# mp3guy/ElasticFusion

Hardware: AMD Instinct MI355X
Metric: frames/s per GPU, 640x480 3-level ICP+fuse (higher is better)
Workload: dtype f32

## Files before the change

### elasticfusion_amd/api.py

```python
from __future__ import annotations

import ctypes as C
import os
import re

import numpy as np

_HERE = os.path.dirname(os.path.abspath(__file__))
LIB_PATH = os.environ.get("EF_HIP_LIB") or os.path.join(_HERE, "libefusion_hip.so")
_lib = None

c_f, c_i, c_u32, P = C.c_float, C.c_int, C.c_uint32, C.c_void_p


class EFError(RuntimeError):
    pass


class ef_config(C.Structure):
    _fields_ = [("width", c_i), ("height", c_i), ("fx", c_f), ("fy", c_f), ("cx", c_f), ("cy", c_f),
                ("time_delta", c_i), ("confidence", c_f), ("depth_cut", c_f), ("icp_weight", c_f),
                ("fast_odom", c_i), ("so3", c_i), ("frame_to_frame_rgb", c_i), ("pyramid", c_i), ("rgb_only", c_i),
                ("close_loops", c_i), ("max_surfels", c_u32), ("device", c_i), ("stream", P)]

# ... 1521 lines not shown
        return tmp.to_array(np.float32, (h, w, 4)), vm.to_array(np.float32, (3 * h, w)), nm.to_array(np.float32, (3 * h, w))

    @staticmethod
    def resize_map(src, normalize, init=None):
        h3, w = src.shape
        s = DevBuf.from_array(src)
        o = DevBuf.from_array(np.zeros((h3 // 2, w // 2), np.float32) if init is None else init)
        fn = lib().ef_op_resize_nmap if normalize else lib().ef_op_resize_vmap
        _chk(fn(s.p, w, h3 // 3, o.p, None))
        return o.to_array(np.float32, (h3 // 2, w // 2))

    @staticmethod
    def pyr_down_gauss_f(src):
        return ops._image_op("pyr_down_gauss_f", src, np.float32, 2)

    @staticmethod
    def pyr_down_uchar_gauss(src):
        return ops._image_op("pyr_down_uchar_gauss", src, np.uint8, 2)

    @staticmethod
    def vertices_to_depth(vmaps_tmp, cutoff):
        return ops._image_op("vertices_to_depth", ops._f32(vmaps_tmp), np.float32, 1, cutoff)

    @staticmethod
    def bgr_to_intensity(rgba):
        return ops._image_op("image_bgr_to_intensity", rgba, np.uint8, 1)

    @staticmethod
    def derivative_images(img):
        h, w = img.shape
        s, dx, dy = DevBuf.from_array(img), DevBuf(h * w * 2), DevBuf(h * w * 2)
        _chk(lib().ef_op_compute_derivative_images(s.p, w, h, dx.p, dy.p, None))
        return dx.to_array(np.int16, (h, w)), dy.to_array(np.int16, (h, w))

    @staticmethod
    def project_to_point_cloud(depth, fx, fy, cx, cy, level=0):
        h, w = depth.shape
        s, d = DevBuf.from_array(depth), DevBuf(h * w * 12)
        k = ef_intr(fx, fy, cx, cy)
        _chk(lib().ef_op_project_to_point_cloud(s.p, w, h, C.byref(k), level, d.p, None))
        return d.to_array(np.float32, (h, w, 3))

    @staticmethod
    def icp_step(Rcurr, tcurr, vmap_curr, nmap_curr, Rprev_inv, tprev, intr, vmap_g_prev, nmap_g_prev, distThres, angleThres):
        h3, w = vmap_curr.shape
        bufs = [DevBuf.from_array(a) for a in (vmap_curr, nmap_curr, vmap_g_prev, nmap_g_prev)]
        A, b, res = np.zeros((6, 6), np.float32), np.zeros(6, np.float32), np.zeros(2, np.float32)
        k = ef_intr(*intr)
        _chk(lib().ef_op_icp_step(_ptr(ops._f32(Rcurr).reshape(9)), _ptr(ops._f32(tcurr)), bufs[0].p, bufs[1].p,
                                  _ptr(ops._f32(Rprev_inv).reshape(9)), _ptr(ops._f32(tprev)), C.byref(k), bufs[2].p, bufs[3].p,
                                  distThres, angleThres, w, h3 // 3, _ptr(A), _ptr(b), _ptr(res), None))
        return A, b, res

    @staticmethod
    def rgb_residual(minScale, dIdx, dIdy, lastDepth, nextDepth, lastImage, nextImage, maxDepthDelta, kt, krkinv):
        h, w = nextImage.shape
        bufs = [DevBuf.from_array(a) for a in (dIdx, dIdy, lastDepth, nextDepth, lastImage, nextImage)]
        corres = DevBuf(h * w * 16)
        sigma, count = c_i(0), c_i(0)
        _chk(lib().ef_op_compute_rgb_residual(minScale, bufs[0].p, bufs[1].p, bufs[2].p, bufs[3].p, bufs[4].p, bufs[5].p, corres.p,
                                              maxDepthDelta, _ptr(ops._f32(kt)), _ptr(ops._f32(krkinv).reshape(9)), w, h,
                                              C.byref(sigma), C.byref(count), None))
        return corres.to_array(DATATERM, (h, w)), sigma.value, count.value

    @staticmethod
    def rgb_step(corres, sigma, cloud, fx, fy, dIdx, dIdy, sobelScale):
        h, w = corres.shape
        bufs = [DevBuf.from_array(a) for a in (corres, ops._f32(cloud), dIdx, dIdy)]
        A, b = np.zeros((6, 6), np.float32), np.zeros(6, np.float32)
        _chk(lib().ef_op_rgb_step(bufs[0].p, sigma, bufs[1].p, fx, fy, bufs[2].p, bufs[3].p, sobelScale, w, h,
                                  _ptr(A), _ptr(b), None))
        return A, b

    @staticmethod
    def so3_step(lastImage, nextImage, imageBasis, kinv, krlr):
        h, w = nextImage.shape
        li, ni = DevBuf.from_array(lastImage), DevBuf.from_array(nextImage)
        A, b, res = np.zeros((3, 3), np.float32), np.zeros(3, np.float32), np.zeros(2, np.float32)
        _chk(lib().ef_op_so3_step(li.p, ni.p, _ptr(ops._f32(imageBasis).reshape(9)), _ptr(ops._f32(kinv).reshape(9)),
                                  _ptr(ops._f32(krlr).reshape(9)), w, h, _ptr(A), _ptr(b), _ptr(res), None))
        return A, b, res

    @staticmethod
    def model_maps(pred_vertex, pred_normal, fill_vertex, fill_normal, R, t, maxDepthRGB=6.0, pred_image=None, fill_image=None, camera_frame=False,
                   force_fill_image=False, tally=False, dense_count=0, dense_samples=1, joint=False, raw=None, rgb=None, depth_cut=3.0, init=None):
        h, w, _ = pred_vertex.shape
        init = init or {}
        keep = [DevBuf.from_array(ops._f32(a)) for a in (pred_vertex, pred_normal, fill_vertex, fill_normal)]
        a = ef_model_maps_op()
        a.cols, a.rows = w, h
        a.pred_vertex, a.pred_normal, a.fill_vertex, a.fill_normal = (b.p for b in keep)
        if pred_image is not None:
            imgs = [DevBuf.from_array(np.ascontiguousarray(i, np.uint8)) for i in (pred_image, fill_image)]
            keep += imgs
            a.pred_image, a.fill_image = imgs[0].p, imgs[1].p
        a.R[:] = [float(v) for v in ops._f32(R).reshape(9)]
        a.t[:] = [float(v) for v in ops._f32(t).reshape(3)]
        a.max_depth_rgb = float(maxDepthRGB)
        a.camera_frame, a.force_fill_image, a.tally = int(camera_frame), int(force_fill_image), int(tally)
        a.dense_count, a.dense_samples = int(dense_count), int(dense_samples)
        spec = {}
        for l in range(3):
            spec[f"vmap{l}"] = spec[f"nmap{l}"] = (np.float32, (3 * (h >> l), w >> l))
        spec["depth0"], spec["last0"] = (np.float32, (h, w)), (np.uint8, (h, w))
        if joint:
            spec.update(filtered=(np.uint16, (h, w)), metric=(np.float32, (h, w)), metric_filtered=(np.float32, (h, w)), next0=(np.uint8, (h, w)))
        out = {}
        for name, (dt, shp) in spec.items():
            start = np.zeros(shp, dt) if name not in init else np.ascontiguousarray(init[name], dt)
            assert start.shape == shp, (name, start.shape, shp)
            out[name] = DevBuf.from_array(start)
        for l in range(3):
            a.vmap[l], a.nmap[l] = out[f"vmap{l}"].p, out[f"nmap{l}"].p
        a.depth0, a.last0 = out["depth0"].p, out["last0"].p
        if joint:
            fr = [DevBuf.from_array(np.ascontiguousarray(raw, np.uint16)), DevBuf.from_array(np.ascontiguousarray(rgb, np.uint8))]
            assert raw.shape == (h, w) and rgb.shape == (h, w, 3)
            keep += fr
            a.joint, a.raw, a.rgb3, a.depth_cut = 1, fr[0].p, fr[1].p, float(depth_cut)
            a.filtered, a.metric, a.metric_filtered, a.next0 = (out[n].p for n in ("filtered", "metric", "metric_filtered", "next0"))
        left = C.c_uint(0)
        _chk(lib().ef_op_model_maps(C.byref(a), C.byref(left), None))
        res = {name: out[name].to_array(*spec[name]) for name in spec}
        res["dense_count"] = int(left.value)
        return res

    @staticmethod
    def sobel_mask(nextImage, nextDepth):
        h, w = nextImage[0].shape
        img = [DevBuf.from_array(np.ascontiguousarray(a, np.uint8)) for a in nextImage]
        dep = [DevBuf.from_array(ops._f32(a)) for a in nextDepth]
        for l in range(3):
            assert nextImage[l].shape == nextDepth[l].shape == (h >> l, w >> l), (l, nextImage[l].shape, nextDepth[l].shape)
        outs = [[DevBuf((h >> l) * (w >> l) * sz, fill=0xA5) for l in range(3)] for sz in (2, 2, 1, 4)]
        arr = lambda bufs: (P * 3)(*[b.p for b in bufs])
        _chk(lib().ef_op_sobel_mask(arr(img), arr(dep), w, h, arr(outs[0]), arr(outs[1]), arr(outs[2]), arr(outs[3]), None))
        return tuple([b.to_array(dt, (h >> l, w >> l)) for l, b in enumerate(bufs)] for bufs, dt in zip(outs, (np.int16, np.int16, np.uint8, np.uint32)))

    @staticmethod
    def clean_deform(cam, T_wc, time, idx, vc, ct, nr, confThreshold, timeDelta, maxDepth, surfels, newUnstable, graph, depth, isFern=0):
        s = ops._f32(surfels).reshape(-1, 12)
        nu = ops._f32(newUnstable).reshape(-1, 12)
        g = ops._f32(graph).reshape(-1, 16)
        bufs = [DevBuf.from_array(a) for a in (idx, ops._f32(vc), ops._f32(ct), ops._f32(nr), g, ops._f32(depth))]
        sb, nb = DevBuf.from_array(s), DevBuf.from_array(nu if len(nu) else np.zeros((1, 12), np.float32))
        out = DevBuf((len(s) + len(nu) + 1) * 48)
        n = c_u32(0)
        _chk(lib().ef_op_clean_deform(C.byref(cam), _ptr(ops._T(T_wc)), time, bufs[0].p, bufs[1].p, bufs[2].p, bufs[3].p,
                                      confThreshold, timeDelta, maxDepth, sb.p, len(s), nb.p, len(nu),
                                      bufs[4].p, len(g), bufs[5].p, int(isFern), out.p, C.byref(n), None))
        return out.to_array(np.float32, (n.value, 12))

    LINALG = dict(ldlt6=0, ldlt3f=1, polar3=2, rodrigues=3, se3_inverse=4, se3_log_norm=5, scalar=6, ldlt6_wave=7, ldlt6_every_lane=8,
                  mat_to_quat=9, se3_mul=10, se3_castf=11, se3_inverse_f=12, m4_affine_inverse=13, ldlt_pivots=14, lu_inverse6=15)

    @staticmethod
    def linalg(which, vec, n_out):
        v = np.ascontiguousarray(np.asarray(vec, np.float64).reshape(-1))
        out = np.zeros(n_out, np.float64)
        _chk(lib().ef_op_linalg(ops.LINALG[which], _ptr(v), v.size, _ptr(out), n_out))
        return out

    GN_STATE = ("Rcurr", "tcurr", "resultRt", "krkinv", "kt", "lastRGBErrorLevel", "rgb_broken")

    @staticmethod
    def gn_update(sums, prev, Rprev, tprev, count, sigma, icp, rgb, rgbOnly, icpWeight, knext, level_changes, split_tail, lastA, lastb, stats):
        a = ef_gn_update_args()
        a.sums[:] = [float(v) for v in ops._f32(sums).reshape(58)]
        for name in ("Rcurr", "tcurr", "krkinv", "kt"):
            getattr(a.prev, name)[:] = [float(v) for v in ops._f32(prev[name]).reshape(-1)]
        a.prev.resultRt[:] = [float(v) for v in np.asarray(prev["resultRt"], np.float64).reshape(16)]
        a.prev.lastRGBErrorLevel, a.prev.rgb_broken = float(np.float32(prev["lastRGBErrorLevel"])), int(prev["rgb_broken"])
        a.Rprev[:] = [float(v) for v in ops._f32(Rprev).reshape(9)]
        a.tprev[:] = [float(v) for v in ops._f32(tprev).reshape(3)]
        a.count, a.sigma, a.icp, a.rgb, a.rgb_only = int(count), int(sigma), int(icp), int(rgb), int(rgbOnly)
        a.icp_weight, a.knext, a.level_changes, a.split_tail = float(icpWeight), ef_intr(*[float(v) for v in knext]), int(level_changes), int(split_tail)
        nxt = ef_gn_state()
        A = np.ascontiguousarray(np.asarray(lastA, np.float64).reshape(36)).copy()
        b = np.ascontiguousarray(np.asarray(lastb, np.float64).reshape(6)).copy()
        st = ops._f32(stats).reshape(4).copy()
        _chk(lib().ef_op_gn_update(C.byref(a), C.byref(nxt), _ptr(A), _ptr(b), _ptr(st)))
        out = {n: np.array(getattr(nxt, n)) for n in ("Rcurr", "tcurr", "resultRt", "krkinv", "kt")}
        out["lastRGBErrorLevel"], out["rgb_broken"] = np.float32(nxt.lastRGBErrorLevel), int(nxt.rgb_broken)
        return out, A, b, st

    @staticmethod
    def track_end_tail(Rcurr, tcurr, Rprev, tprev, q_prev, t_prev, rgb, weightMultiplier):
        o = ef_track_end_out()
        qp = np.ascontiguousarray(np.asarray(q_prev, np.float64).reshape(4))
        tp = np.ascontiguousarray(np.asarray(t_prev, np.float64).reshape(3))
        _chk(lib().ef_op_track_end_tail(_ptr(ops._f32(Rcurr).reshape(9)), _ptr(ops._f32(tcurr).reshape(3)), _ptr(ops._f32(Rprev).reshape(9)),
                                        _ptr(ops._f32(tprev).reshape(3)), _ptr(qp), _ptr(tp), int(rgb), weightMultiplier, C.byref(o)))
        out = {n: np.array(getattr(o, n)) for n in ("q", "t", "logged", "T_cw", "pose_f", "R_wc_f", "t_wc_f")}
        out["weighting"] = np.float32(o.weighting)
        return out

    @staticmethod
    def filter_depth(raw, maxD):
        return ops._image_op("filter_depth", raw, np.uint16, 1, maxD)

    @staticmethod
    def metricise_depth(d_in, maxD):
        return ops._image_op("metricise_depth", d_in, np.float32, 1, maxD)

    @staticmethod
    def seed_map(cam, rgb, dm, dmf, time, maxDepth):
        Pn = cam.cols * cam.rows
        bufs = [DevBuf.from_array(a) for a in (rgb, dm, dmf)]
        out = DevBuf(Pn * 48)
        n = c_u32(0)
        _chk(lib().ef_op_seed_map(C.byref(cam), bufs[0].p, bufs[1].p, bufs[2].p, time, maxDepth, out.p, C.byref(n), None))
        return out.to_array(np.float32, (n.value, 12))

    @staticmethod
    def _T(T):
        return np.ascontiguousarray(T, np.float64).reshape(16)

    @staticmethod
    def predict_indices(cam, T_wc, time, surfels, maxDepth, timeDelta):
        s = ops._f32(surfels).reshape(-1, 12)
        Pn = cam.cols * cam.rows
        sb = DevBuf.from_array(s)
        idx, vc, ct, nr = DevBuf(Pn * 4), DevBuf(Pn * 16), DevBuf(Pn * 16), DevBuf(Pn * 16)
        _chk(lib().ef_op_predict_indices(C.byref(cam), _ptr(ops._T(T_wc)), time, sb.p, len(s), maxDepth, timeDelta,
                                         idx.p, vc.p, ct.p, nr.p, None))
        shp = (cam.rows, cam.cols)
        return (idx.to_array(np.uint32, shp), vc.to_array(np.float32, shp + (4,)), ct.to_array(np.float32, shp + (4,)),
                nr.to_array(np.float32, shp + (4,)))

    @staticmethod
    def combined_predict(cam, T_wc, surfels, maxDepth, confThreshold, time, maxTime, timeDelta):
        s = ops._f32(surfels).reshape(-1, 12)
        Pn = cam.cols * cam.rows
        sb = DevBuf.from_array(s)
        img, vt, nm, tm = DevBuf(Pn * 4), DevBuf(Pn * 16), DevBuf(Pn * 16), DevBuf(Pn * 2)
        _chk(lib().ef_op_combined_predict(C.byref(cam), _ptr(ops._T(T_wc)), sb.p, len(s), maxDepth, confThreshold,
                                          time, maxTime, timeDelta, img.p, vt.p, nm.p, tm.p, None))
        shp = (cam.rows, cam.cols)
        return (img.to_array(np.uint8, shp + (4,)), vt.to_array(np.float32, shp + (4,)), nm.to_array(np.float32, shp + (4,)),
                tm.to_array(np.uint16, shp))

    @staticmethod
    def synthesize_depth(cam, T_wc, surfels, maxDepth, confThreshold, time, maxTime, timeDelta):
        s = ops._f32(surfels).reshape(-1, 12)
        Pn = cam.cols * cam.rows
        sb, d = DevBuf.from_array(s), DevBuf(Pn * 4)
        _chk(lib().ef_op_synthesize_depth(C.byref(cam), _ptr(ops._T(T_wc)), sb.p, len(s), maxDepth, confThreshold,
                                          time, maxTime, timeDelta, d.p, None))
        return d.to_array(np.float32, (cam.rows, cam.cols))

    @staticmethod
    def fill_in(cam, image, vertex, normal, depthFiltered, rgb, passthrough=0, passthroughImage=0):
        bufs = [DevBuf.from_array(a) for a in (image, ops._f32(vertex), ops._f32(normal), depthFiltered, rgb)]
        Pn = cam.cols * cam.rows
        fi, fv, fn = DevBuf(Pn * 4), DevBuf(Pn * 16), DevBuf(Pn * 16)
        _chk(lib().ef_op_fill_in(C.byref(cam), bufs[0].p, bufs[1].p, bufs[2].p, bufs[3].p, bufs[4].p, passthrough, passthroughImage,
                                 fi.p, fv.p, fn.p, None))
        shp = (cam.rows, cam.cols)
        return fi.to_array(np.uint8, shp + (4,)), fv.to_array(np.float32, shp + (4,)), fn.to_array(np.float32, shp + (4,))

    @staticmethod
    def dense_enough(cam, image):
        b = DevBuf.from_array(image)
        d = c_i(0)
        _chk(lib().ef_op_dense_enough(C.byref(cam), b.p, C.byref(d), None))
        return bool(d.value)

    @staticmethod
    def fuse(cam, T_wc, time, rgb, dm, dmf, idx, vc, ct, nr, maxDepth, weighting, surfels):
        s = ops._f32(surfels).reshape(-1, 12)
        bufs = [DevBuf.from_array(a) for a in (rgb, dm, dmf, idx, ops._f32(vc), ops._f32(ct), ops._f32(nr))]
        sb = DevBuf.from_array(s)
        nu = DevBuf((cam.cols // 2) * (cam.rows // 2) * 48)
        n = c_u32(0)
        _chk(lib().ef_op_fuse(C.byref(cam), _ptr(ops._T(T_wc)), time, bufs[0].p, bufs[1].p, bufs[2].p, bufs[3].p, bufs[4].p, bufs[5].p,
                              bufs[6].p, maxDepth, weighting, sb.p, len(s), nu.p, C.byref(n), None))
        return sb.to_array(np.float32, (len(s), 12)), nu.to_array(np.float32, (n.value, 12))

    @staticmethod
    def clean(cam, T_wc, time, idx, vc, ct, nr, confThreshold, timeDelta, maxDepth, surfels, newUnstable):
        s = ops._f32(surfels).reshape(-1, 12)
        nu = ops._f32(newUnstable).reshape(-1, 12)
        bufs = [DevBuf.from_array(a) for a in (idx, ops._f32(vc), ops._f32(ct), ops._f32(nr))]
        sb, nb = DevBuf.from_array(s), DevBuf.from_array(nu if len(nu) else np.zeros((1, 12), np.float32))
        out = DevBuf((len(s) + len(nu) + 1) * 48)
        n = c_u32(0)
        _chk(lib().ef_op_clean(C.byref(cam), _ptr(ops._T(T_wc)), time, bufs[0].p, bufs[1].p, bufs[2].p, bufs[3].p, confThreshold,
                               timeDelta, maxDepth, sb.p, len(s), nb.p, len(nu), out.p, C.byref(n), None))
        return out.to_array(np.float32, (n.value, 12))
```

### elasticfusion_amd/csrc/ef_host_ops.inc

```
extern "C" {

__global__ void k_calib_empty() {}
__global__ void __launch_bounds__(256) k_calib_stream(const float4* __restrict__ src, float4* __restrict__ dst, int n) {
  for (int i = blockIdx.x * blockDim.x + threadIdx.x; i < n; i += gridDim.x * blockDim.x) dst[i] = src[i];
}
int ef_dev_calibrate(void* stream, float* empty_us, float* stream16mb_us) {
  if (!empty_us || !stream16mb_us) return EF_EINVAL;
  hipStream_t s = (hipStream_t)stream;
  const int n = 1 << 20, reps = 200;
  float4 *a = nullptr, *b = nullptr;
  hipEvent_t e0 = nullptr, e1 = nullptr;
  int rc = EF_EHIP;
  float ms = 0;
  if (hipMalloc((void**)&a, (size_t)n * sizeof(float4)) != hipSuccess || hipMalloc((void**)&b, (size_t)n * sizeof(float4)) != hipSuccess) { rc = EF_ENOMEM; goto done; }
  if (hipMemsetAsync(a, 0, (size_t)n * sizeof(float4), s) != hipSuccess) goto done;
  if (hipEventCreate(&e0) != hipSuccess || hipEventCreate(&e1) != hipSuccess) goto done;
  for (int pass = 0; pass < 2; ++pass) {
    if (hipEventRecord(e0, s) != hipSuccess) goto done;
    for (int i = 0; i < reps; ++i) hipLaunchKernelGGL(k_calib_empty, dim3(256), dim3(256), 0, s);
    if (hipEventRecord(e1, s) != hipSuccess || hipEventSynchronize(e1) != hipSuccess || hipEventElapsedTime(&ms, e0, e1) != hipSuccess) goto done;
    *empty_us = 1e3f * ms / reps;
    if (hipEventRecord(e0, s) != hipSuccess) goto done;
    for (int i = 0; i < reps; ++i) hipLaunchKernelGGL(k_calib_stream, dim3(2048), dim3(256), 0, s, (const float4*)a, b, n);
    if (hipEventRecord(e1, s) != hipSuccess || hipEventSynchronize(e1) != hipSuccess || hipEventElapsedTime(&ms, e0, e1) != hipSuccess) goto done;
// ... 52 lines not shown
  eft::copy_maps(v4, n4, cols, rows, tmp, vd, nd, (hipStream_t)s);
  OP_TAIL(s);
}
int ef_op_resize_vmap(const float* in, int sc, int sr, float* out, void* s) { eft::resize_map(in, sc, sr, out, false, (hipStream_t)s); OP_TAIL(s); }
int ef_op_resize_nmap(const float* in, int sc, int sr, float* out, void* s) { eft::resize_map(in, sc, sr, out, true, (hipStream_t)s); OP_TAIL(s); }
int ef_op_pyr_down_gauss_f(const float* src, int sc, int sr, float* dst, void* s) { eft::pyr_down_gauss_f(src, sc, sr, dst, (hipStream_t)s); OP_TAIL(s); }
int ef_op_pyr_down_uchar_gauss(const uint8_t* src, int sc, int sr, uint8_t* dst, void* s) { eft::pyr_down_uchar_gauss(src, sc, sr, dst, (hipStream_t)s); OP_TAIL(s); }
int ef_op_vertices_to_depth(const float* tmp, int cols, int rows, float cutoff, float* dst, void* s) { eft::vertices_to_depth(tmp, cols, rows, cutoff, dst, (hipStream_t)s); OP_TAIL(s); }
int ef_op_image_bgr_to_intensity(const uint8_t* rgba, int cols, int rows, uint8_t* dst, void* s) { eft::bgr_to_intensity(rgba, 4, cols, rows, dst, (hipStream_t)s); OP_TAIL(s); }
int ef_op_compute_derivative_images(const uint8_t* src, int cols, int rows, int16_t* dx, int16_t* dy, void* s) {
  eft::derivative_images(src, cols, rows, dx, dy, (hipStream_t)s);
  OP_TAIL(s);
}
int ef_op_project_to_point_cloud(const float* depth, int cols, int rows, const ef_intr* k0, int level, float* cloud, void* s) {
  eft::project_to_point_cloud(depth, cols, rows, eft::intr_level(eft::Intr{k0->fx, k0->fy, k0->cx, k0->cy}, level), cloud, (hipStream_t)s);
  OP_TAIL(s);
}

static int op_scratch(float** partials, float** out, int nfloats_out) {
  if (hipMalloc((void**)partials, (size_t)eft::OP_SCRATCH_FLOATS * sizeof(float)) != hipSuccess) return EF_ENOMEM;
  if (hipMalloc((void**)out, nfloats_out * sizeof(float)) != hipSuccess) { (void)hipFree(*partials); return EF_ENOMEM; }
  return EF_OK;
}
static void unpack29_host(const float* h, float* A, float* b) {
  int shift = 0;
  for (int i = 0; i < 6; ++i)
    for (int j = i; j < 7; ++j) {
      const float v = h[shift++];
      if (j == 6) b[i] = v;
      else A[j * 6 + i] = A[i * 6 + j] = v;
    }
}
int ef_op_icp_step(const float* Rc, const float* tc, const float* vc, const float* nc, const float* Rpi, const float* tp, const ef_intr* k,
                   const float* vg, const float* ng, float dist, float ang, int cols, int rows, float* A, float* b, float* res, void* s) {
  if (cols <= 0 || rows <= 0 || cols > 2048 || rows > 2048) return EF_EINVAL;
  eft::IcpArgs a;
  memcpy(a.Rcurr, Rc, 36); memcpy(a.tcurr, tc, 12); memcpy(a.Rprev_inv, Rpi, 36); memcpy(a.tprev, tp, 12);
  a.k = eft::Intr{k->fx, k->fy, k->cx, k->cy};
  a.distThres = dist; a.angleThres = ang;
  float *partials, *out;
  int r = op_scratch(&partials, &out, 32);
  if (r != EF_OK) return r;
  eft::icp_step_op(a, vc, nc, vg, ng, cols, rows, partials, out, (hipStream_t)s);
  float h[32];
  (void)hipMemcpyAsync(h, out, 29 * sizeof(float), hipMemcpyDeviceToHost, (hipStream_t)s);
  hipError_t e = hipStreamSynchronize((hipStream_t)s);
  (void)hipFree(partials); (void)hipFree(out);
  if (e != hipSuccess) { g_create_error = hipGetErrorString(e); return EF_EHIP; }
  unpack29_host(h, A, b);
  res[0] = h[27]; res[1] = h[28];
  return EF_OK;
}
int ef_op_compute_rgb_residual(float minScale, const int16_t* dIdx, const int16_t* dIdy, const float* lastDepth, const float* nextDepth,
                               const uint8_t* lastImage, const uint8_t* nextImage, void* corres, float maxDepthDelta, const float* kt,
                               const float* krkinv, int cols, int rows, int* sigma, int* count, void* s) {
  eft::RgbResidualArgs a;
  a.minScale = minScale; a.maxDepthDelta = maxDepthDelta;
  memcpy(a.kt, kt, 12); memcpy(a.krkinv, krkinv, 36);
  int* out;
  if (hipMalloc((void**)&out, 2 * sizeof(int)) != hipSuccess) return EF_ENOMEM;
  eft::rgb_residual_op(a, dIdx, dIdy, lastDepth, nextDepth, lastImage, nextImage, corres, cols, rows, out, (hipStream_t)s);
  int h[2] = {0, 0};
  hipError_t e = hipMemcpy(h, out, sizeof(h), hipMemcpyDeviceToHost);
  (void)hipFree(out);
  if (e != hipSuccess) { g_create_error = hipGetErrorString(e); return EF_EHIP; }
  *count = h[0];
  *sigma = h[1];
  return EF_OK;
}
int ef_op_rgb_step(const void* corres, float sigma, const float* cloud, float fx, float fy, const int16_t* dIdx, const int16_t* dIdy,
                   float sobelScale, int cols, int rows, float* A, float* b, void* s) {
  float *partials, *out;
  int r = op_scratch(&partials, &out, 32);
  if (r != EF_OK) return r;
  eft::rgb_step_op(corres, sigma, cloud, fx, fy, dIdx, dIdy, sobelScale, cols, rows, partials, out, (hipStream_t)s);
  float h[32];
  (void)hipMemcpyAsync(h, out, 29 * sizeof(float), hipMemcpyDeviceToHost, (hipStream_t)s);
  hipError_t e = hipStreamSynchronize((hipStream_t)s);
  (void)hipFree(partials); (void)hipFree(out);
  if (e != hipSuccess) { g_create_error = hipGetErrorString(e); return EF_EHIP; }
  unpack29_host(h, A, b);
  return EF_OK;
}
int ef_op_so3_step(const uint8_t* lastImage, const uint8_t* nextImage, const float* ib, const float* kinv, const float* krlr, int cols,
                   int rows, float* A, float* b, float* res, void* s) {
  eft::So3Args a;
  memcpy(a.imageBasis, ib, 36); memcpy(a.kinv, kinv, 36); memcpy(a.krlr, krlr, 36);
  float *partials, *out;
  int r = op_scratch(&partials, &out, 16);
  if (r != EF_OK) return r;
  eft::so3_step_op(a, lastImage, nextImage, cols, rows, partials, out, (hipStream_t)s);
  float h[11];
  (void)hipMemcpyAsync(h, out, sizeof(h), hipMemcpyDeviceToHost, (hipStream_t)s);
  hipError_t e = hipStreamSynchronize((hipStream_t)s);
  (void)hipFree(partials); (void)hipFree(out);
  if (e != hipSuccess) { g_create_error = hipGetErrorString(e); return EF_EHIP; }
  int shift = 0;
  for (int i = 0; i < 3; ++i)
    for (int j = i; j < 4; ++j) {
      const float v = h[shift++];
      if (j == 3) b[i] = v;
      else A[j * 3 + i] = A[i * 3 + j] = v;
    }
  res[0] = h[9]; res[1] = h[10];
  return EF_OK;
}

int ef_op_model_maps(const ef_model_maps_op* a, unsigned* dense_count_left, void* s) {
  if (!a || !dense_count_left || a->cols <= 0 || a->rows <= 0 || a->cols > 2048 || a->rows > 2048 || (a->cols & 3) || (a->rows & 3)) return EF_EINVAL;
  if (!a->pred_vertex || !a->pred_normal || !a->fill_vertex || !a->fill_normal || !a->depth0) return EF_EINVAL;
  if ((a->pred_image == nullptr) != (a->fill_image == nullptr) || (a->pred_image && !a->last0)) return EF_EINVAL;
  for (int i = 0; i < eft::NUM_PYRS; ++i)
    if (!a->vmap[i] || !a->nmap[i]) return EF_EINVAL;
  if (a->joint && (!a->raw || !a->rgb3 || !a->filtered || !a->metric || !a->metric_filtered || !a->next0)) return EF_EINVAL;
  eft::ModelMapsOp o{};
  o.cols = a->cols; o.rows = a->rows;
  o.pred_vertex = a->pred_vertex; o.pred_normal = a->pred_normal; o.fill_vertex = a->fill_vertex; o.fill_normal = a->fill_normal;
  o.pred_image = a->pred_image; o.fill_image = a->fill_image;
  memcpy(o.R, a->R, 36); memcpy(o.t, a->t, 12);
  o.maxDepthRGB = a->max_depth_rgb;
  o.camera_frame = a->camera_frame != 0; o.force_fill_image = a->force_fill_image != 0; o.tally = a->tally != 0;
  o.dense_count = a->dense_count; o.dense_samples = a->dense_samples;
  for (int i = 0; i < eft::NUM_PYRS; ++i) { o.vmap[i] = a->vmap[i]; o.nmap[i] = a->nmap[i]; }
  o.depth0 = a->depth0; o.last0 = a->last0;
  eft::FramePreprocess fp{};
  if (a->joint) {
    fp = eft::FramePreprocess{a->raw, a->depth_cut, efm::bilateral_table(), a->filtered, a->metric, a->metric_filtered, a->rgb3, nullptr};
    if (!fp.table) { g_create_error = "bilateral weight table missing on this device"; return EF_EHIP; }
    o.with = &fp; o.next0 = a->next0;
  }
  const hipError_t e = (hipError_t)eft::model_maps_op(o, dense_count_left, (hipStream_t)s);
  if (e != hipSuccess) { g_create_error = hipGetErrorString(e); return e == hipErrorOutOfMemory ? EF_ENOMEM : EF_EHIP; }
  return EF_OK;
}
int ef_op_sobel_mask(const uint8_t* const* nextImage, const float* const* nextDepth, int cols, int rows, int16_t* const* dIdx, int16_t* const* dIdy,
                     uint8_t* const* mask, uint32_t* const* corres, void* s) {
  if (!nextImage || !nextDepth || !dIdx || !dIdy || !mask || !corres || cols <= 0 || rows <= 0 || cols > 2048 || rows > 2048) return EF_EINVAL;
  eft::SobelMaskOp o{};
  o.cols = cols; o.rows = rows;
  for (int i = 0; i < eft::NUM_PYRS; ++i) {
    if (!nextImage[i] || !nextDepth[i] || !dIdx[i] || !dIdy[i] || !mask[i] || !corres[i]) return EF_EINVAL;
    o.nextImage[i] = nextImage[i]; o.nextDepth[i] = nextDepth[i]; o.dIdx[i] = dIdx[i]; o.dIdy[i] = dIdy[i]; o.mask[i] = mask[i]; o.corres[i] = corres[i];
  }
  eft::sobel_mask_op(o, (hipStream_t)s);
  const hipError_t le = hipGetLastError();
  if (le != hipSuccess) { g_create_error = hipGetErrorString(le); return EF_EHIP; }
  OP_SYNC(s);
  return EF_OK;
}

}
namespace {
__global__ void k_linalg_probe(int which, const double* __restrict__ in, double* __restrict__ out) {
  if (which == EF_LINALG_LDLT6_WAVE || which == EF_LINALG_LDLT6_EVERY_LANE) {
    __shared__ efs::SolveScratch S;
    const int lane = threadIdx.x;
    if (lane < 6) S.b[lane] = in[36 + lane];
    efs::wave_sync();
    if (which == EF_LINALG_LDLT6_WAVE) efs::ldlt6_wave(in[lane < 36 ? lane : 0], S);
    else efs::ldlt6_every_lane(in[lane < 36 ? lane : 0], S);
    if (lane < 6) out[lane] = S.x[lane];
    return;
  }
  if (threadIdx.x != 0) return;
  switch (which) {
    case EF_LINALG_LDLT6: efl::ldlt_solve<double, 6>(in, in + 36, out); break;
    case EF_LINALG_LDLT3F: {
      float A[9], b[3], x[3];
      for (int i = 0; i < 9; ++i) A[i] = (float)in[i];
      for (int i = 0; i < 3; ++i) b[i] = (float)in[9 + i];
      efl::ldlt_solve<float, 3>(A, b, x);
      for (int i = 0; i < 3; ++i) out[i] = (double)x[i];
      break;
    }
    case EF_LINALG_POLAR3: efl::polar3(in, out); break;
    case EF_LINALG_RODRIGUES: efl::rodrigues(in, out); break;
    case EF_LINALG_SE3_INVERSE: efl::se3_matrix(efl::se3_inverse(efl::se3_from_matrix(in)), out); break;
    case EF_LINALG_SE3_LOG_NORM: out[0] = efl::se3_log_norm(efl::se3_from_matrix(in)); break;
    case EF_LINALG_SCALAR:
      out[0] = sqrt(in[0]); out[1] = in[0] / in[1]; out[2] = sin(in[0]); out[3] = cos(in[0]); out[4] = atan2(in[0], in[1]);
      break;
    case EF_LINALG_MAT_TO_QUAT: {
      efl::mat_to_quat(in, out);
      efl::SE3 T;
      efl::se3_set_rotation(T, in);
      for (int i = 0; i < 4; ++i) out[4 + i] = T.q[i];
      break;
    }
    case EF_LINALG_SE3_MUL: {
      const efl::SE3 T = efl::se3_mul(efl::se3_from_matrix(in), efl::se3_from_matrix(in + 16));
      for (int i = 0; i < 4; ++i) out[i] = T.q[i];
      for (int i = 0; i < 3; ++i) out[4 + i] = T.t[i];
      break;
    }
    case EF_LINALG_SE3_CASTF:
    case EF_LINALG_SE3_INVERSE_F: {
      float M[16];
      if (which == EF_LINALG_SE3_CASTF) efl::se3_castf_matrix(efl::se3_from_matrix(in), M);
      else efl::se3_inverse_matrix_f(efl::se3_from_matrix(in), M);
      for (int i = 0; i < 16; ++i) out[i] = (double)M[i];
      break;
    }
    case EF_LINALG_M4_AFFINE_INVERSE: efl::m4_affine_inverse(in, out); break;
    case EF_LINALG_LDLT_PIVOTS: efl::ldlt_pivots<double, 6>(in, out); break;
    case EF_LINALG_LU_INVERSE6: efl::lu_inverse<double, 6>(in, out); break;
    default: break;
  }
}
}
extern "C" {
int ef_op_linalg(int which, const double* in, int n_in, double* out, int n_out) {
  if (!in || !out || n_in <= 0 || n_out <= 0 || n_in > 64 || n_out > 64 || which < 0 || which > EF_LINALG_LU_INVERSE6) return EF_EINVAL;
  double* d;
  if (hipMalloc((void**)&d, 128 * sizeof(double)) != hipSuccess) return EF_ENOMEM;
  (void)hipMemset(d, 0, 128 * sizeof(double));
  (void)hipMemcpy(d, in, n_in * sizeof(double), hipMemcpyHostToDevice);
  hipLaunchKernelGGL(k_linalg_probe, dim3(1), dim3(64), 0, 0, which, (const double*)d, d + 64);
  hipError_t e = hipMemcpy(out, d + 64, n_out * sizeof(double), hipMemcpyDeviceToHost);
  (void)hipFree(d);
  if (e != hipSuccess) { g_create_error = hipGetErrorString(e); return EF_EHIP; }
  return EF_OK;
}

static_assert(sizeof(ef_gn_state) == sizeof(eft::GNState), "ef_gn_state is eft::GNState");
int ef_op_gn_update(const ef_gn_update_args* in, ef_gn_state* next, double* lastA36, double* lastb6, float* stats4) {
  if (!in || !next || !lastA36 || !lastb6 || !stats4 || !(in->icp || in->rgb)) return EF_EINVAL;
  eft::GnUpdateProbe p;
  memcpy(p.sums, in->sums, sizeof(p.sums));
  memcpy(&p.prev, &in->prev, sizeof(p.prev));
  memcpy(p.Rprev, in->Rprev, 36); memcpy(p.tprev, in->tprev, 12);
  p.count = in->count; p.sigma = in->sigma;
  p.icp = in->icp != 0; p.rgb = in->rgb != 0; p.rgbOnly = in->rgb_only != 0;
  p.icpWeight = in->icp_weight;
  p.knext = eft::Intr{in->knext.fx, in->knext.fy, in->knext.cx, in->knext.cy};
  p.level_changes = in->level_changes != 0;
  p.split_tail = in->split_tail != 0;
  const hipError_t e = (hipError_t)eft::gn_update_op(p, (eft::GNState*)next, lastA36, lastb6, stats4);
  if (e != hipSuccess) { g_create_error = hipGetErrorString(e); return e == hipErrorOutOfMemory ? EF_ENOMEM : EF_EHIP; }
  return EF_OK;
}
int ef_op_track_end_tail(const float* Rcurr9, const float* tcurr3, const float* Rprev9, const float* tprev3, const double* q_prev4,
                         const double* t_prev3, int rgb, float weight_multiplier, ef_track_end_out* out) {
  if (!Rcurr9 || !tcurr3 || !Rprev9 || !tprev3 || !q_prev4 || !t_prev3 || !out) return EF_EINVAL;
  eft::TrackState* st = new eft::TrackState();
  memcpy(st->Rprev, Rprev9, 36); memcpy(st->tprev, tprev3, 12);
  memcpy(st->q_prev, q_prev4, 32); memcpy(st->t_prev, t_prev3, 24);
  float pose[12];
  memcpy(pose, Rcurr9, 36); memcpy(pose + 9, tcurr3, 12);
  const hipError_t e = (hipError_t)eft::track_end_tail_op(st, pose, rgb != 0, weight_multiplier, out->logged);
  if (e == hipSuccess) {
    memcpy(out->q, st->q, 32); memcpy(out->t, st->t, 24);
    memcpy(out->T_cw, st->T_cw, 64); memcpy(out->pose_f, st->pose_f, 64);
    memcpy(out->R_wc_f, st->R_wc_f, 36); memcpy(out->t_wc_f, st->t_wc_f, 12);
    out->weighting = st->weighting;
  }
  delete st;
  if (e != hipSuccess) { g_create_error = hipGetErrorString(e); return e == hipErrorOutOfMemory ? EF_ENOMEM : EF_EHIP; }
  return EF_OK;
}

int ef_op_filter_depth(const uint16_t* raw, int cols, int rows, float maxD, uint16_t* filtered, void* s) {
  if (!efm::filter_depth(raw, cols, rows, maxD, filtered, (hipStream_t)s)) return EF_EHIP;
  OP_TAIL(s);
}
int ef_op_metricise_depth(const uint16_t* in, int cols, int rows, float maxD, float* out, void* s) {
  efm::metricise_depth(in, cols, rows, maxD, out, (hipStream_t)s);
  OP_TAIL(s);
}

}
namespace {
struct OpMap {
  std::vector<void*> allocs;
  template <typename T>
  T* alloc(size_t n, int fill = 0) {
    void* p = nullptr;
    if (hipMalloc(&p, (n ? n : 1) * sizeof(T)) != hipSuccess) return nullptr;
    (void)hipMemset(p, fill, (n ? n : 1) * sizeof(T));
    allocs.push_back(p);
    return (T*)p;
  }
  efm::SurfelSoA soa(size_t n) { return efm::SurfelSoA{alloc<float4>(n), alloc<float4>(n), alloc<float4>(n)}; }
  ~OpMap() { for (void* p : allocs) (void)hipFree(p); }
};
efm::Cam to_cam(const ef_cam* c) { return efm::Cam{c->cols, c->rows, c->fx, c->fy, c->cx, c->cy}; }
}
extern "C" {

int ef_op_seed_map(const ef_cam* cam, const uint8_t* rgb, const float* dm, const float* dmf, int time, float maxDepth, float* surfels,
                   uint32_t* count_host, void* s_) {
  hipStream_t s = (hipStream_t)s_;
  OpMap m;
  const size_t P = (size_t)cam->cols * cam->rows;
  efm::SurfelSoA soa = m.soa(P);
  efm::CompactScratch cs;
  cs.max_chunks = (int)(2 * P / efm::CHUNK + 8);
  cs.flags = m.alloc<uint8_t>(2 * P);
  cs.chunk_count = m.alloc<uint32_t>(cs.max_chunks);
  cs.chunk_offset = m.alloc<uint32_t>(cs.max_chunks);
  cs.totals = m.alloc<uint32_t>(8);
  unsigned* cnt = m.alloc<unsigned>(1);
  efm::seed_map(to_cam(cam), rgb, dm, dmf, time, maxDepth, soa, cnt, cs, s);
  unsigned h = 0;
  (void)hipMemcpyAsync(&h, cnt, sizeof(h), hipMemcpyDeviceToHost, s);
  OP_SYNC(s);
  efm::soa_to_aos(soa, h, surfels, s);
  OP_SYNC(s);
  *count_host = h;
  return EF_OK;
}

int ef_op_predict_indices(const ef_cam* cam, const double* T16, int time, const float* surfels, uint32_t count, float maxDepth, int timeDelta,
                          uint32_t* index, float* vc, float* ct, float* nr, void* s_) {
  hipStream_t s = (hipStream_t)s_;
  OpMap m;
  const size_t P = (size_t)cam->cols * cam->rows;
  efm::SurfelSoA soa = m.soa(count);
  efm::aos_to_soa(surfels, count, soa, s);
  float h[32];
  pose_mats(T16, h, h + 16);
  float* mats = m.alloc<float>(32);
  (void)hipMemcpyAsync(mats, h, sizeof(h), hipMemcpyHostToDevice, s);
  unsigned* cnt = m.alloc<unsigned>(1);
  (void)hipMemcpyAsync(cnt, &count, sizeof(unsigned), hipMemcpyHostToDevice, s);
  unsigned long long* zbuf = m.alloc<unsigned long long>(P, 0xFF);
  efm::IndexMaps im{index, (float4*)vc, (float4*)ct, (float4*)nr};
  efm::predict_indices(to_cam(cam), mats, time, soa, cnt, maxDepth, timeDelta, zbuf, im, s);
  OP_SYNC(s);
  return EF_OK;
}

int ef_op_combined_predict(const ef_cam* cam, const double* T16, const float* surfels, uint32_t count, float maxDepth, float confThreshold,
                           int time, int maxTime, int timeDelta, uint8_t* image, float* vertex, float* normal, uint16_t* timeMap, void* s_) {
  hipStream_t s = (hipStream_t)s_;
  OpMap m;
  const size_t P = (size_t)cam->cols * cam->rows;
  efm::SurfelSoA soa = m.soa(count);
  efm::aos_to_soa(surfels, count, soa, s);
  float h[32];
  pose_mats(T16, h, h + 16);
  float* mats = m.alloc<float>(32);
  (void)hipMemcpyAsync(mats, h, sizeof(h), hipMemcpyHostToDevice, s);
  unsigned* cnt = m.alloc<unsigned>(1);
  (void)hipMemcpyAsync(cnt, &count, sizeof(unsigned), hipMemcpyHostToDevice, s);
  unsigned long long* zbuf = m.alloc<unsigned long long>(P, 0xFF);
  efm::PredictMaps pm{(uchar4*)image, (float4*)vertex, (float4*)normal, timeMap};
  efm::FillMaps none{nullptr, nullptr, nullptr};
  efm::combined_predict(to_cam(cam), mats, soa, cnt, maxDepth, confThreshold, time, maxTime, timeDelta, zbuf, pm, none, nullptr, nullptr, false,
                        nullptr, s);
  OP_SYNC(s);
  return EF_OK;
}

int ef_op_synthesize_depth(const ef_cam* cam, const double* T16, const float* surfels, uint32_t count, float maxDepth, float confThreshold,
                           int time, int maxTime, int timeDelta, float* depth, void* s_) {
  hipStream_t s = (hipStream_t)s_;
  OpMap m;
  const size_t P = (size_t)cam->cols * cam->rows;
  efm::SurfelSoA soa = m.soa(count);
  efm::aos_to_soa(surfels, count, soa, s);
  float h[32];
  pose_mats(T16, h, h + 16);
  float* mats = m.alloc<float>(32);
  (void)hipMemcpyAsync(mats, h, sizeof(h), hipMemcpyHostToDevice, s);
  unsigned* cnt = m.alloc<unsigned>(1);
  (void)hipMemcpyAsync(cnt, &count, sizeof(unsigned), hipMemcpyHostToDevice, s);
  unsigned long long* zbuf = m.alloc<unsigned long long>(P, 0xFF);
  efm::synthesize_depth(to_cam(cam), mats, soa, cnt, maxDepth, confThreshold, time, maxTime, timeDelta, zbuf, depth, s);
  OP_SYNC(s);
  return EF_OK;
}

int ef_op_fill_in(const ef_cam* cam, const uint8_t* image, const float* vertex, const float* normal, const uint16_t* depthFiltered,
                  const uint8_t* rgb, int passthrough, int passthroughImage, uint8_t* fimage, float* fvertex, float* fnormal, void* s_) {
  efm::PredictMaps pm{(uchar4*)image, (float4*)vertex, (float4*)normal, nullptr};
  efm::FillMaps fm{(uchar4*)fimage, (float4*)fvertex, (float4*)fnormal};
  efm::fill_in(to_cam(cam), pm, depthFiltered, rgb, passthrough != 0, passthroughImage != 0, fm, (hipStream_t)s_);
  OP_TAIL(s_);
}

int ef_op_dense_enough(const ef_cam* cam, const uint8_t* image, int* dense_host, void* s_) {
  hipStream_t s = (hipStream_t)s_;
  OpMap m;
  unsigned* cnt = m.alloc<unsigned>(1);
  efm::dense_count(to_cam(cam), (const uchar4*)image, cnt, s);
  unsigned h = 0;
  (void)hipMemcpyAsync(&h, cnt, sizeof(h), hipMemcpyDeviceToHost, s);
  OP_SYNC(s);
  *dense_host = ((float)h / (float)((cam->cols / 20) * (cam->rows / 20)) > 0.75f) ? 1 : 0;
// ... 108 lines not shown
```

### elasticfusion_amd/csrc/ef_solve_dev.hpp

```cpp
#pragma once
#include <hip/hip_runtime.h>
#include <float.h>
#include "ef_linalg_dev.hpp"
#include "ef_track.hpp"

namespace efs {

#ifdef EF_STAGE_CLOCKS
#define EF_STAMP(st, i) do { if ((threadIdx.x & 63) == 0 && blockIdx.x == 0) (st)->dbg_clock[i] = wall_clock64(); } while (0)
#else
#define EF_STAMP(st, i) do { } while (0)
#endif

__device__ __forceinline__ void wave_sync() {
  __builtin_amdgcn_fence(__ATOMIC_RELEASE, "wavefront");
  __builtin_amdgcn_wave_barrier();
  __builtin_amdgcn_fence(__ATOMIC_ACQUIRE, "wavefront");
}
__device__ __forceinline__ double shfl_d(double v, int src) { return __shfl(v, src, 64); }
__device__ __forceinline__ double bcast_d(double v, int src) {
  return __hiloint2double(__builtin_amdgcn_readlane(__double2hiint(v), src), __builtin_amdgcn_readlane(__double2loint(v), src));
}

struct SolveScratch {
  double A[36];
  double b[6];
  double x[6];
  double upd[16];
  double Rt[16];
  double inv[2][9];
  double ti[3];
  double KR[9];
  float pose[12];
  double prevRt[16];
  float prevPose[12];
  float krkinv[9], kt[3];
  float Rcurr[9], tcurr[3];
  int broken;
  int tail_pending;
};
struct SolvePrefetch {
  double rt;
  float pose;
  int slot_a, slot_b;
  float lastRGBErrorLevel;
  int broken;
};
__device__ __forceinline__ SolvePrefetch solve_prefetch(const eft::TrackState* st, const eft::GNState* prev, const int* slots) {
  const int lane = threadIdx.x & 63;
  SolvePrefetch P;
  P.rt = prev->resultRt[lane & 15];
  P.pose = lane < 9 ? st->Rprev[lane] : st->tprev[lane < 12 ? lane - 9 : 0];
  P.slot_a = slots[lane * 16];
  P.slot_b = slots[lane * 16 + 1];
  P.lastRGBErrorLevel = prev->lastRGBErrorLevel;
  P.broken = prev->rgb_broken;
  return P;
}
__device__ __forceinline__ void solve_prefetch_publish(const SolvePrefetch& P, SolveScratch& S) {
  const int lane = threadIdx.x & 63;
  if (lane < 16) S.prevRt[lane] = P.rt;
  if (lane < 12) S.prevPose[lane] = P.pose;
}

__device__ __forceinline__ int se3_member_of(int i, int j) {
  const int lo = i < j ? i : j, hi = i < j ? j : i;
  const int start = lo * 7 - (lo * (lo - 1)) / 2;
  return start + (hi - lo);
}

__device__ __forceinline__ void ldlt6_wave(double a, SolveScratch& S) {
  const int lane = threadIdx.x & 63;
  const int e = lane < 36 ? lane : 0;
  const int i = e / 6, j = e - i * 6;
  const int hi = i > j ? i : j, lo = i > j ? j : i;
  int perm[6] = {0, 1, 2, 3, 4, 5};
#pragma unroll
  for (int k = 0; k < 6; ++k) {
    int p = k;
    double best = fabs(bcast_d(a, k * 7));
#pragma unroll
    for (int m = k + 1; m < 6; ++m) {
      const double v = fabs(bcast_d(a, m * 7));
      const bool gt = v > best;
      best = gt ? v : best;
      p = gt ? m : p;
    }
    const int pi = (i == k) ? p : ((i == p) ? k : i);
    const int pj = (j == k) ? p : ((j == p) ? k : j);
    a = shfl_d(a, pi * 6 + pj);
#pragma unroll
    for (int m = k + 1; m < 6; ++m) {
      const bool sw = (p == m);
      const int pk = perm[k], pm = perm[m];
      perm[k] = sw ? pm : pk;
      perm[m] = sw ? pk : pm;
    }
    const double d = bcast_d(a, k * 7);
    const double c_hi = shfl_d(a, hi * 6 + k), c_lo = shfl_d(a, lo * 6 + k);
    if (!(d == 0.0)) {
      const double l = c_hi / d;
      if (i > k && j > k) a = a - l * c_lo;
      else if (j == k && i > k) a = l;
      else if (i == k && j > k) a = 0.0;
    }
  }
  if (lane < 36) S.A[lane] = a;
  wave_sync();
  double F[36];
#pragma unroll
  for (int q = 0; q < 36; ++q) F[q] = S.A[q];
  double y[6];
#pragma unroll
  for (int q = 0; q < 6; ++q) y[q] = S.b[perm[q]];
#pragma unroll
  for (int r = 0; r < 6; ++r)
#pragma unroll
    for (int c = 0; c < r; ++c) y[r] -= F[r * 6 + c] * y[c];
#pragma unroll
  for (int r = 0; r < 6; ++r) {
    const double d = F[r * 7];
    y[r] = (fabs(d) > DBL_MIN) ? y[r] / d : 0.0;
  }
#pragma unroll
  for (int r = 5; r >= 0; --r)
#pragma unroll
    for (int c = r + 1; c < 6; ++c) y[r] -= F[c * 6 + r] * y[c];
  if (lane == 0) {
#pragma unroll
    for (int q = 0; q < 6; ++q) S.x[perm[q]] = y[q];
  }
  wave_sync();
}

__device__ __forceinline__ double m3_inverse_entry(const double* m, int e) {
  double o[9];
  efl::m3_inverse<double>(m, o);
  double r = o[0];
#pragma unroll
  for (int q = 1; q < 9; ++q) r = (e == q) ? o[q] : r;
  return r;
}

__device__ __forceinline__ constexpr int ldlt6_at(int i, int j) { return i >= j ? i * (i + 1) / 2 + j : j * (j + 1) / 2 + i; }
template <int K, int M_>
__device__ __forceinline__ void ldlt6_swap(double (&A)[21], unsigned& perm ) {
  double B[21];
#pragma unroll
  for (int i = 0; i < 6; ++i)
#pragma unroll
    for (int j = 0; j <= i; ++j) {
      const int pi = (i == K) ? M_ : ((i == M_) ? K : i), pj = (j == K) ? M_ : ((j == M_) ? K : j);
      B[ldlt6_at(i, j)] = A[ldlt6_at(pi, pj)];
    }
#pragma unroll
  for (int q = 0; q < 21; ++q) A[q] = B[q];
  const unsigned pk = (perm >> (3 * K)) & 7u, pm = (perm >> (3 * M_)) & 7u;
  perm = (perm & ~((7u << (3 * K)) | (7u << (3 * M_)))) | (pm << (3 * K)) | (pk << (3 * M_));
}
template <int K>
__device__ __forceinline__ void ldlt6_step(double (&A)[21], unsigned& perm) {
  int p = K;
  double best = fabs(A[ldlt6_at(K, K)]);
#pragma unroll
  for (int m = K + 1; m < 6; ++m) {
    const double v = fabs(A[ldlt6_at(m, m)]);
    const bool gt = v > best;
    best = gt ? v : best;
    p = gt ? m : p;
  }
  p = __builtin_amdgcn_readfirstlane(p);
  if (K + 1 < 6 && p == K + 1) ldlt6_swap<K, (K + 1 < 6 ? K + 1 : K)>(A, perm);
  else if (K + 2 < 6 && p == K + 2) ldlt6_swap<K, (K + 2 < 6 ? K + 2 : K)>(A, perm);
  else if (K + 3 < 6 && p == K + 3) ldlt6_swap<K, (K + 3 < 6 ? K + 3 : K)>(A, perm);
  else if (K + 4 < 6 && p == K + 4) ldlt6_swap<K, (K + 4 < 6 ? K + 4 : K)>(A, perm);
  else if (K + 5 < 6 && p == K + 5) ldlt6_swap<K, (K + 5 < 6 ? K + 5 : K)>(A, perm);
  const double d = A[ldlt6_at(K, K)];
  if (!(d == 0.0)) {
    double colk[6];
#pragma unroll
    for (int i = K + 1; i < 6; ++i) colk[i] = A[ldlt6_at(i, K)];
#pragma unroll
    for (int i = K + 1; i < 6; ++i) {
      const double l = colk[i] / d;
#pragma unroll
      for (int j = K + 1; j <= i; ++j) A[ldlt6_at(i, j)] = A[ldlt6_at(i, j)] - l * colk[j];
      A[ldlt6_at(i, K)] = l;
    }
  }
}
__device__ __forceinline__ void ldlt6_every_lane(double a, SolveScratch& S) {
  const int lane = threadIdx.x & 63;
  if (lane < 36) S.A[lane] = a;
  wave_sync();
  double A[21];
#pragma unroll
  for (int i = 0; i < 6; ++i)
#pragma unroll
    for (int j = 0; j <= i; ++j) A[ldlt6_at(i, j)] = S.A[i * 6 + j];
  unsigned perm = 0u | (1u << 3) | (2u << 6) | (3u << 9) | (4u << 12) | (5u << 15);
  ldlt6_step<0>(A, perm);
  ldlt6_step<1>(A, perm);
  ldlt6_step<2>(A, perm);
  ldlt6_step<3>(A, perm);
  ldlt6_step<4>(A, perm);
  ldlt6_step<5>(A, perm);
  double y[6];
#pragma unroll
  for (int q = 0; q < 6; ++q) y[q] = S.b[(perm >> (3 * q)) & 7u];
#pragma unroll
  for (int r = 0; r < 6; ++r)
#pragma unroll
    for (int c = 0; c < r; ++c) y[r] -= A[ldlt6_at(r, c)] * y[c];
#pragma unroll
  for (int r = 0; r < 6; ++r) {
    const double d = A[ldlt6_at(r, r)];
    y[r] = (fabs(d) > DBL_MIN) ? y[r] / d : 0.0;
  }
#pragma unroll
  for (int r = 5; r >= 0; --r)
#pragma unroll
    for (int c = r + 1; c < 6; ++c) y[r] -= A[ldlt6_at(c, r)] * y[c];
  if (lane == 0) {
#pragma unroll
    for (int q = 0; q < 6; ++q) S.x[(perm >> (3 * q)) & 7u] = y[q];
  }
  wave_sync();
}

struct SolveInputs {
  bool icp, rgb, rgbOnly;
  float icpWeight;
  eft::Intr knext;
  bool level_changes;
};

__device__ __forceinline__ void gn_tail_pose(SolveScratch& S, eft::GNState* next, bool publish) {
  const int lane = threadIdx.x & 63;
  if (lane < 12) {
    float iR[9], ot[3], it[3];
#pragma unroll
    for (int r = 0; r < 3; ++r) {
#pragma unroll
      for (int c = 0; c < 3; ++c) iR[r * 3 + c] = (float)S.Rt[c * 4 + r];
      ot[r] = (float)S.Rt[r * 4 + 3];
    }
#pragma unroll
    for (int r = 0; r < 3; ++r) it[r] = -(iR[r * 3] * ot[0] + iR[r * 3 + 1] * ot[1] + iR[r * 3 + 2] * ot[2]);
    const float* Rp = S.prevPose;
    if (lane < 9) {
      const int r = lane / 3, c = lane - r * 3;
      const float i0 = (float)S.Rt[c * 4], i1 = (float)S.Rt[c * 4 + 1], i2 = (float)S.Rt[c * 4 + 2];
      const float v = Rp[r * 3] * i0 + Rp[r * 3 + 1] * i1 + Rp[r * 3 + 2] * i2;
      S.Rcurr[lane] = v;
      if (publish) next->Rcurr[lane] = v;
    } else {
      const int r = lane - 9;
      const float v = (Rp[r * 3] * it[0] + Rp[r * 3 + 1] * it[1] + Rp[r * 3 + 2] * it[2]) + S.prevPose[9 + r];
      S.tcurr[r] = v;
      if (publish) next->tcurr[r] = v;
    }
  }
}
__device__ __forceinline__ void gn_tail_krk(const eft::Intr knext, SolveScratch& S, eft::GNState* next, bool publish) {
  const int lane = threadIdx.x & 63;
  {
    const eft::Intr k = knext;
    const double K[9] = {k.fx, 0, k.cx, 0, k.fy, k.cy, 0, 0, 1};
    const bool second = lane >= 16;
    double m[9];
#pragma unroll
    for (int q = 0; q < 9; ++q) m[q] = second ? K[q] : S.Rt[(q / 3) * 4 + (q % 3)];
    const int e = second ? lane - 16 : lane;
    const double inv = m3_inverse_entry(m, (e >= 0 && e < 9) ? e : 0);
    if (lane < 9) S.inv[0][lane] = inv;
    else if (lane >= 16 && lane < 25) S.inv[1][lane - 16] = inv;
    wave_sync();
    if (lane < 3) {
      const double* Ai = S.inv[0];
      S.ti[lane] = Ai[lane * 3] * S.Rt[3] + Ai[lane * 3 + 1] * S.Rt[7] + Ai[lane * 3 + 2] * S.Rt[11];
    }
    if (lane >= 16 && lane < 25) {
      const int q = lane - 16, r = q / 3, c = q - r * 3;
      const double k0 = (r == 0) ? K[0] : 0.0, k1 = (r == 1) ? K[4] : 0.0, k2 = (r == 0) ? K[2] : (r == 1 ? K[5] : 1.0);
      double s = 0;
      s += k0 * S.inv[0][c];
      s += k1 * S.inv[0][3 + c];
      s += k2 * S.inv[0][6 + c];
      S.KR[q] = s;
    }
    wave_sync();
    if (lane < 9) {
      const int r = lane / 3, c = lane - r * 3;
      double s = 0;
#pragma unroll
      for (int kk = 0; kk < 3; ++kk) s += S.KR[r * 3 + kk] * S.inv[1][kk * 3 + c];
      S.krkinv[lane] = (float)s;
      if (publish) next->krkinv[lane] = (float)s;
    } else if (lane >= 16 && lane < 19) {
      const int r = lane - 16;
      const double t0 = -S.ti[0], t1 = -S.ti[1], t2 = -S.ti[2];
      const double k0 = (r == 0) ? K[0] : 0.0, k1 = (r == 1) ? K[4] : 0.0, k2 = (r == 0) ? K[2] : (r == 1 ? K[5] : 1.0);
      const float v = (float)(k0 * t0 + k1 * t1 + k2 * t2);
      S.kt[r] = v;
      if (publish) next->kt[r] = v;
    }
  }
  wave_sync();
}
template <bool SPLIT_TAIL = false>
__device__ __forceinline__ void gauss_newton_update_wave(eft::TrackState* st, eft::GNState* next, bool publish, const float* sums,
                                                         const SolveInputs in, SolveScratch& S, bool stats) {
  const int lane = threadIdx.x & 63;
  double a = 0.0;
  {
    const int e = lane < 36 ? lane : 0;
    const int i = e / 6, j = e - i * 6;
    const int mA = se3_member_of(i, j);
    const int bi = lane >= 36 && lane < 42 ? lane - 36 : 0;
    const int mb = se3_member_of(bi, 6);
    const int m = lane < 36 ? mA : mb;
    double v;
    if (in.icp && in.rgb) {
      const double w = in.icpWeight;
      if (lane < 36) v = (double)sums[eft::SE3_ACCS + m] + w * w * (double)sums[m];
      else v = (double)sums[eft::SE3_ACCS + m] + w * (double)sums[m];
    } else if (in.icp) {
      v = (double)sums[m];
    } else {
      v = (double)sums[eft::SE3_ACCS + m];
    }
    if (lane < 36) { a = v; if (stats) st->lastA[lane] = v; }
    else if (lane < 42) { S.b[lane - 36] = v; if (stats) st->lastb[lane - 36] = v; }
  }
  wave_sync();
  EF_STAMP(st, 4);
  ldlt6_every_lane(a, S);
  EF_STAMP(st, 5);
  {
    double rx = S.x[3], ry = S.x[4], rz = S.x[5];
    const double theta = sqrt(rx * rx + ry * ry + rz * rz);
    double val;
    const int e = lane < 16 ? lane : 0;
    const int r = e >> 2, c = e & 3;
    if (r < 3 && c < 3) {
      const int k = r * 3 + c;
      val = (r == c) ? 1.0 : 0.0;
      if (theta >= DBL_EPSILON) {
#ifdef __HIP_DEVICE_COMPILE__
        double sn, cs;
        sincos(theta, &sn, &cs);
        const double c1 = 1. - cs;
#else
        const double cs = cos(theta), sn = sin(theta), c1 = 1. - cs;
#endif
        const double itheta = theta ? 1. / theta : 0.;
        rx *= itheta; ry *= itheta; rz *= itheta;
        const double u = (r == 0) ? rx : (r == 1 ? ry : rz), v = (c == 0) ? rx : (c == 1 ? ry : rz);
        const double rrt = (r <= c) ? u * v : v * u;
        double cross = 0.0;
        if (k == 1) cross = -rz; else if (k == 2) cross = ry; else if (k == 3) cross = rz;
        else if (k == 5) cross = -rx; else if (k == 6) cross = -ry; else if (k == 7) cross = rx;
        val = cs * ((r == c) ? 1.0 : 0.0) + c1 * rrt + sn * cross;
      }
    } else if (r < 3) {
      val = S.x[r];
    } else {
      val = (c == 3) ? 1.0 : 0.0;
    }
    if (lane < 16) S.upd[lane] = val;
  }
  wave_sync();
  EF_STAMP(st, 6);
  if (lane < 16) {
    const int r = lane >> 2, c = lane & 3;
    double s = 0;
#pragma unroll
    for (int k = 0; k < 4; ++k) s += S.upd[r * 4 + k] * S.prevRt[k * 4 + c];
    S.Rt[lane] = s;
  }
  wave_sync();
  if (publish && lane < 16) next->resultRt[lane] = S.Rt[lane];
  if (SPLIT_TAIL) {
    if (lane == 0) S.tail_pending = 1;
    wave_sync();
    return;
  }
  gn_tail_pose(S, next, publish);
  EF_STAMP(st, 7);
  gn_tail_krk(in.knext, S, next, publish);
  wave_sync();
  EF_STAMP(st, 8);
}

}
```

### elasticfusion_amd/csrc/ef_track.hpp

```cpp
#pragma once
#include <hip/hip_runtime.h>
#include <stdint.h>

#include "ef_build.hpp"

namespace eft {

constexpr int NUM_PYRS = 3;
constexpr int REDUCE_BLOCK = 256;
constexpr int VTHREADS = 16384;
constexpr int VWARPS = VTHREADS / 32;
constexpr int RGB_SLOTS = 64;
constexpr int SE3_ACCS = 29;
constexpr int SO3_ACCS = 11;
constexpr int SE3_PAIRS = VWARPS / 2;
constexpr int PARTIAL_FLOATS = 2 * SE3_ACCS * SE3_PAIRS > SO3_ACCS * VWARPS ? 2 * SE3_ACCS * SE3_PAIRS : SO3_ACCS * VWARPS;
constexpr int PT_WGS = 128, PT_BLOCK = 512, PT_MAX_ITER = 16, PT_MAX_PIXELS = 8 * VTHREADS, PT_SYNC_FLOATS = 1024;
constexpr int PARTIAL_ALLOC_FLOATS = (2 * PARTIAL_FLOATS + PT_SYNC_FLOATS) > 196608 ? (2 * PARTIAL_FLOATS + PT_SYNC_FLOATS) : 196608;
constexpr int FT_EPOCHS = 64;

struct Intr { float fx, fy, cx, cy; };
__host__ __device__ inline Intr intr_level(const Intr& k, int level) {
  const int div = 1 << level;
  return Intr{k.fx / div, k.fy / div, k.cx / div, k.cy / div};
}

struct GNState {
  float Rcurr[9], tcurr[3];
  double resultRt[16];
  float krkinv[9], kt[3];
  float lastRGBErrorLevel;
  int rgb_broken;
};

struct TrackState {
  double q[4];
  double t[3];
  double q_prev[4];
  double t_prev[3];
  float Rprev[9], tprev[3], Rprev_inv[9];
  GNState gn[2];
  int rgb_slots[2][RGB_SLOTS][16];
  float lastICPError, lastICPCount, lastRGBError, lastRGBCount, lastSO3Error, lastSO3Count;
  double lastA[36], lastb[6];
  int so3_iterations;
  double so3_resultR[9], so3_lastResultR[9];
  float so3_R_lr[9];
  float so3_mats[27];
  float so3_lastError, so3_lastCount;
  int so3_done;
  unsigned so3_ticket;
  float weighting;
  unsigned dense_count;
  int dense_samples;
  int tick;
  unsigned long long step_rec[16];
  unsigned call_seq;
  unsigned step_timeout;
  unsigned long long dbg_clock[16];
  unsigned map_counts[2];
  unsigned model_view_stamp;
  float T_cw[16];
  float pose_f[16];
  float R_wc_f[9], t_wc_f[3];
};

struct TrackerPlan {
  int script = 0;
  int n_small = 0;
  int n_iter = 0;
  unsigned long long levels = 0;
  unsigned res_bytes = 0;
  unsigned res_budget = 0;
};

struct Pyramid {
  int width, height;
  uint16_t* depth_tmp[NUM_PYRS];
  float* vmap_curr[NUM_PYRS];
  float* nmap_curr[NUM_PYRS];
  float* vmap_g_prev[NUM_PYRS];
  float* nmap_g_prev[NUM_PYRS];
  float* lastDepth[NUM_PYRS];
  float* nextDepth[NUM_PYRS];
  uint8_t* lastImage[NUM_PYRS];
  uint8_t* nextImage[NUM_PYRS];
  uint8_t* lastNextImage[NUM_PYRS];
  int16_t* dIdx[NUM_PYRS];
  int16_t* dIdy[NUM_PYRS];
  uint32_t* corres[NUM_PYRS];
  uint8_t* rgbMask[NUM_PYRS];
  float* partials;
  unsigned epoch = 1;
  int last_mode = 0;
  unsigned sticky_abort = 0, fallbacks_base = 0;
  TrackerPlan plan;
  int W(int l) const { return width >> l; }
  int H(int l) const { return height >> l; }
};

struct KernelProbe {
  hipEvent_t* start;
  hipEvent_t* stop;
  int capacity;
  int used;
};

struct TrackParams {
  bool rgbOnly, pyramid, fastOdom, so3;
  float icpWeight;
  float distThres, angleThres;
  int fused_step = 0;
  int persistent = 1;
  const unsigned* empty_model_flag = nullptr;
  unsigned empty_model_value = 0;
  int no_resident = 0;
};
static_assert(sizeof(TrackParams) == 4 + 4 + 8 + 4 + 4 + 8 + 4 + 4, "TrackParams has no padding bytes (it is compared with memcmp)");

void pyr_down_u16(const uint16_t* src, int scols, int srows, uint16_t* dst, hipStream_t s);
void create_vmap(const uint16_t* depth, int cols, int rows, Intr k, float cutoff, float* vmap, hipStream_t s);
void create_nmap(const float* vmap, int cols, int rows, float* nmap, hipStream_t s);
void transform_maps(const float* vsrc, const float* nsrc, int cols, int rows, const float* R9_dev, const float* t3_dev,
                    float* vdst, float* ndst, hipStream_t s);
void copy_maps(const float* vtex, const float* ntex, int cols, int rows, float* vmaps_tmp, float* vmap, float* nmap, hipStream_t s);
void resize_map(const float* in, int scols, int srows, float* out, bool normalize, hipStream_t s);
void pyr_down_gauss_f(const float* src, int scols, int srows, float* dst, hipStream_t s);
void pyr_down_uchar_gauss(const uint8_t* src, int scols, int srows, uint8_t* dst, hipStream_t s);
void vertices_to_depth(const float* vmaps_tmp, int cols, int rows, float cutoff, float* dst, hipStream_t s);
void bgr_to_intensity(const uint8_t* src, int channels, int cols, int rows, uint8_t* dst, hipStream_t s);
void derivative_images(const uint8_t* src, int cols, int rows, int16_t* dx, int16_t* dy, hipStream_t s);
void project_to_point_cloud(const float* depth, int cols, int rows, Intr k, float* cloud, hipStream_t s);

struct IcpArgs {
  float Rcurr[9], tcurr[3], Rprev_inv[9], tprev[3];
  Intr k;
  float distThres, angleThres;
};
constexpr int OP_SCRATCH_FLOATS = SE3_ACCS * VWARPS + 64;
void icp_step_op(const IcpArgs& a, const float* vmap_curr, const float* nmap_curr, const float* vmap_g_prev,
                 const float* nmap_g_prev, int cols, int rows, float* scratch, float* out29_dev, hipStream_t s);
struct RgbResidualArgs {
  float minScale, maxDepthDelta;
  float kt[3], krkinv[9];
};
void rgb_residual_op(const RgbResidualArgs& a, const int16_t* dIdx, const int16_t* dIdy, const float* lastDepth,
                     const float* nextDepth, const uint8_t* lastImage, const uint8_t* nextImage, void* corres, int cols,
                     int rows, int* out2_dev, hipStream_t s);
void rgb_step_op(const void* corres, float sigma, const float* cloud, float fx, float fy, const int16_t* dIdx,
                 const int16_t* dIdy, float sobelScale, int cols, int rows, float* scratch, float* out29_dev, hipStream_t s);
struct So3Args { float imageBasis[9], kinv[9], krlr[9]; };
void so3_step_op(const So3Args& a, const uint8_t* lastImage, const uint8_t* nextImage, int cols, int rows, float* scratch,
                 float* out11_dev, hipStream_t s);

struct GnUpdateProbe {
  float sums[2 * SE3_ACCS];
  GNState prev;
  float Rprev[9], tprev[3];
  int count, sigma;
  bool icp, rgb, rgbOnly;
  float icpWeight;
  Intr knext;
  bool level_changes;
  bool split_tail;
};
int gn_update_op(const GnUpdateProbe& p, GNState* next_host, double* lastA36, double* lastb6, float* stats4);
int track_end_tail_op(TrackState* st_host, const float* pose12, bool rgb, float weightMultiplier, double* logged16);

struct FramePreprocess {
  const uint16_t* raw;
  float maxD;
  const float* table;
  uint16_t* filtered;
  float* metric;
  float* metric_filtered;
  const uint8_t* rgb3;
  uint8_t* rgb_keep;
};
void init_icp_model(const Pyramid& p, const float* pred_vertex, const float* pred_normal, const float* fill_vertex,
                    const float* fill_normal, const TrackState* st, float maxDepthRGB, hipStream_t s, const uint8_t* pred_image_rgba = nullptr,
                    const uint8_t* fill_image_rgba = nullptr, bool frameToFrameRGB = false, const FramePreprocess* with = nullptr,
                    bool tally = false );
void init_icp_maps(const Pyramid& p, const float* vertex4, const float* normal4, const uint8_t* image_rgba, const TrackState* st,
                   float maxDepthRGB, hipStream_t s);
void build_pyramids(const Pyramid& p, const uint16_t* depth_filtered, Intr k, float cutoff, hipStream_t s, bool with_sobel);
void build_pyramids_frame_side(const Pyramid& p, const uint16_t* depth_filtered, Intr k, float cutoff, hipStream_t s);
void build_pyramids_model_side(const Pyramid& p, hipStream_t s);
void init_rgb_sobel(const Pyramid& p, hipStream_t s);
void init_model_pair(const Pyramid& p, const float* model_vertex4, const float* model_normal4, const uint8_t* model_image_rgba,
                     const float* cur_vertex4, const float* cur_normal4, const uint8_t* cur_image_rgba, const TrackState* st, float maxDepthRGB,
                     hipStream_t s);
struct ModelMapsOp {
  int cols, rows;
  const float *pred_vertex, *pred_normal, *fill_vertex, *fill_normal;
  const uint8_t *pred_image, *fill_image;
  float R[9], t[3], maxDepthRGB;
  bool camera_frame, force_fill_image, tally;
  unsigned dense_count;
  int dense_samples;
  float* vmap[NUM_PYRS];
  float* nmap[NUM_PYRS];
  float* depth0;
  uint8_t* last0;
  const FramePreprocess* with;
  uint8_t* next0;
};
int model_maps_op(const ModelMapsOp& o, unsigned* dense_count_left, hipStream_t s);
struct SobelMaskOp {
  int cols, rows;
  const uint8_t* nextImage[NUM_PYRS];
  const float* nextDepth[NUM_PYRS];
  int16_t* dIdx[NUM_PYRS];
  int16_t* dIdy[NUM_PYRS];
  uint8_t* mask[NUM_PYRS];
  uint32_t* corres[NUM_PYRS];
};
void sobel_mask_op(const SobelMaskOp& o, hipStream_t s);
void init_first_rgb(const Pyramid& p, const uint8_t* rgb3, hipStream_t s);
struct TrackTail {
  int cur, slots;
  bool has_head, icp, rgb, rgbOnly;
  float icpWeight;
  Intr k0;
  const float* pairs;
  int ng = 0;
  bool merged_end = false;
  unsigned epoch = 0;
  float* partials = nullptr;
};
TrackTail track(Pyramid& p, TrackState* st, Intr k, const TrackParams& tp, hipStream_t s, KernelProbe* probe = nullptr,
                KernelProbe* probe_all = nullptr);
int tracker_aborted(const Pyramid& p, hipStream_t s);
void track_prepare(Pyramid& p, const TrackParams& tp, hipStream_t s);
int tracker_fallbacks(const Pyramid& p, hipStream_t s);
void persistent_chain_forget(hipStream_t s);
int tracker_small_clocks(const Pyramid& p, unsigned long long* out32, hipStream_t s);
void track_swap(Pyramid& p, const TrackParams& tp);
void track_end(TrackState* st, const TrackTail& tail, bool rgb, float weightMultiplier, double* traj, int slot, hipStream_t s,
               const unsigned* abort_word = nullptr, unsigned* abort_report = nullptr);
unsigned* tracker_abort_word(const Pyramid& p);
void pose_injected(TrackState* st, const double* T_wc16, bool save_prev, float weightMultiplier, bool with_weighting, double* traj,
                   int slot, hipStream_t s);
void log_pose(const TrackState* st, double* traj, int slot, hipStream_t s);
void pose_restored(TrackState* st, const double* q4, const double* t3, hipStream_t s);
void copy_pose(TrackState* dst, const TrackState* src, hipStream_t s);
void adopt_pose(TrackState* st, const TrackState* est, double* traj, int slot, hipStream_t s);
void sample_constraints(const float* vertex4, const uint16_t* old_time, int cols, int rows, int step, float* out4, hipStream_t s);

}
```

### elasticfusion_amd/csrc/ef_track_host_ops.inc

```
namespace {
inline int ceil_div(int a, int b) { return (a + b - 1) / b; }
}

void pyr_down_u16(const uint16_t* src, int scols, int srows, uint16_t* dst, hipStream_t s) {
  hipLaunchKernelGGL(k_pyr_down_u16, tile_grid(scols / 2, srows / 2), tile_block(), 0, s, src, scols, srows, dst);
}
void create_vmap(const uint16_t* depth, int cols, int rows, Intr k, float cutoff, float* vmap, hipStream_t s) {
  hipLaunchKernelGGL(k_create_vmap, tile_grid(cols, rows), tile_block(), 0, s, depth, cols, rows, 1.f / k.fx, 1.f / k.fy, k.cx, k.cy, cutoff, vmap);
}
void create_nmap(const float* vmap, int cols, int rows, float* nmap, hipStream_t s) {
  hipLaunchKernelGGL(k_create_nmap, tile_grid(cols, rows), tile_block(), 0, s, vmap, cols, rows, nmap);
}
void transform_maps(const float* vsrc, const float* nsrc, int cols, int rows, const float* R9_dev, const float* t3_dev, float* vdst,
                    float* ndst, hipStream_t s) {
  hipLaunchKernelGGL(k_transform_maps, tile_grid(cols, rows), tile_block(), 0, s, vsrc, nsrc, cols, rows, R9_dev, t3_dev, vdst, ndst);
}
void copy_maps(const float* vtex, const float* ntex, int cols, int rows, float* vmaps_tmp, float* vmap, float* nmap, hipStream_t s) {
  hipLaunchKernelGGL(k_copy_maps, tile_grid(cols, rows), tile_block(), 0, s, (const float4*)vtex, (const float4*)ntex, cols, rows,
                     (float4*)vmaps_tmp, vmap, nmap);
}
void resize_map(const float* in, int scols, int srows, float* out, bool normalize, hipStream_t s) {
  if (normalize) hipLaunchKernelGGL(k_resize_map<true>, tile_grid(scols / 2, srows / 2), tile_block(), 0, s, in, scols, srows, out);
  else hipLaunchKernelGGL(k_resize_map<false>, tile_grid(scols / 2, srows / 2), tile_block(), 0, s, in, scols, srows, out);
}
void pyr_down_gauss_f(const float* src, int scols, int srows, float* dst, hipStream_t s) {
  hipLaunchKernelGGL(k_pyr_down_gauss_f, tile_grid(scols / 2, srows / 2), tile_block(), 0, s, src, scols, srows, dst);
}
void pyr_down_uchar_gauss(const uint8_t* src, int scols, int srows, uint8_t* dst, hipStream_t s) {
  hipLaunchKernelGGL(k_pyr_down_uchar_gauss, tile_grid(scols / 2, srows / 2), tile_block(), 0, s, src, scols, srows, dst);
}
void vertices_to_depth(const float* vmaps_tmp, int cols, int rows, float cutoff, float* dst, hipStream_t s) {
  hipLaunchKernelGGL(k_vertices_to_depth, tile_grid(cols, rows), tile_block(), 0, s, (const float4*)vmaps_tmp, cols, rows, cutoff, dst);
}
void bgr_to_intensity(const uint8_t* src, int channels, int cols, int rows, uint8_t* dst, hipStream_t s) {
  const int n = cols * rows;
  if (channels == 4) hipLaunchKernelGGL(k_bgr_to_intensity<4>, dim3(ceil_div(n, 256)), dim3(256), 0, s, src, n, dst);
  else hipLaunchKernelGGL(k_bgr_to_intensity<3>, dim3(ceil_div(n, 256)), dim3(256), 0, s, src, n, dst);
}
void derivative_images(const uint8_t* src, int cols, int rows, int16_t* dx, int16_t* dy, hipStream_t s) {
  hipLaunchKernelGGL(k_sobel, tile_grid(cols, rows), tile_block(), 0, s, src, cols, rows, dx, dy);
}
void project_to_point_cloud(const float* depth, int cols, int rows, Intr k, float* cloud, hipStream_t s) {
  hipLaunchKernelGGL(k_project_points, tile_grid(cols, rows), tile_block(), 0, s, depth, cols, rows, 1.0f / k.fx, 1.0f / k.fy, k.cx, k.cy, cloud);
}

namespace {
template <class F>
void with_terms(bool icp, bool rgb, F&& f) {
  if (icp && rgb) f(std::true_type{}, std::true_type{});
  else if (icp) f(std::true_type{}, std::false_type{});
  else f(std::false_type{}, std::true_type{});
}
template <bool HAS_ICP, bool HAS_RGB, bool PACKED>
void launch_accum(const IcpView& IV, const RgbView& RV, const Se3Inputs& in, int N, const Se3Out& out, hipStream_t s, hipEvent_t start = nullptr,
                  hipEvent_t stop = nullptr) {
#ifdef EF_FAST_ORDER
  {
    const FastPlan fp = fast_plan(N);
    const dim3 fgrid(in.xcd_swizzle ? 8 * fast_groups_per_xcd(fp.NG) : fp.NG), fblock(256 * ((HAS_ICP && HAS_RGB) ? 2 : 1));
    hipExtLaunchKernelGGL((k_se3_accum_fast<HAS_ICP, HAS_RGB, PACKED>), fgrid, fblock, 0, s, start, stop, 0, IV, RV, in, out.pairs);
  }
#else
  constexpr int BLOCK = 64 * 2 * ACC_NW * ((HAS_ICP && HAS_RGB) ? 2 : 1);
  const dim3 grid(VWARPS / ACC_NW), block(BLOCK);
#ifdef EF_VISIT_PAIRS
  if (HAS_ICP || PACKED) {
    const int S = ((N + VTHREADS - 1) / VTHREADS + 3) >> 2;
    if (S <= 2) hipExtLaunchKernelGGL((k_se3_accum<2, HAS_ICP, HAS_RGB, PACKED>), grid, block, 0, s, start, stop, 0, IV, RV, in, out);
    else if (S % 6 == 0 || S % 6 == 5 || !(S % 4 == 0 || S % 4 == 3)) hipExtLaunchKernelGGL((k_se3_accum<6, HAS_ICP, HAS_RGB, PACKED>), grid, block, 0, s, start, stop, 0, IV, RV, in, out);
    else hipExtLaunchKernelGGL((k_se3_accum<4, HAS_ICP, HAS_RGB, PACKED>), grid, block, 0, s, start, stop, 0, IV, RV, in, out);
    return;
  }
#endif
  if (N > 8 * VTHREADS) hipExtLaunchKernelGGL((k_se3_accum<5, HAS_ICP, HAS_RGB, PACKED>), grid, block, 0, s, start, stop, 0, IV, RV, in, out);
  else hipExtLaunchKernelGGL((k_se3_accum<2, HAS_ICP, HAS_RGB, PACKED>), grid, block, 0, s, start, stop, 0, IV, RV, in, out);
#endif
}
inline int op_groups(int N) {
#ifdef EF_FAST_ORDER
  return fast_plan(N).NG;
#else
  (void)N;
  return 0;
#endif
}
inline int so3_grid(int N) {
#ifdef EF_FAST_ORDER
  return 8 * fast_groups_per_xcd(fast_plan(N).NG);
#else
  (void)N;
  return VWARPS / SO3_WPB;
#endif
}
}

void icp_step_op(const IcpArgs& a, const float* vmap_curr, const float* nmap_curr, const float* vmap_g_prev,
                 const float* nmap_g_prev, int cols, int rows, float* scratch, float* out29_dev, hipStream_t s) {
  IcpView V{vmap_curr, nmap_curr, vmap_g_prev, nmap_g_prev, cols, rows, a.k, a.distThres, a.angleThres, sq_le_max(a.distThres), sq_lt_max(a.angleThres)};
  RgbView RV{};
  float* pose = scratch + SE3_ACCS * VWARPS;
  float h[24];
  for (int i = 0; i < 9; ++i) { h[i] = a.Rcurr[i]; h[12 + i] = a.Rprev_inv[i]; }
  for (int i = 0; i < 3; ++i) { h[9 + i] = a.tcurr[i]; h[21 + i] = a.tprev[i]; }
  (void)hipMemcpyAsync(pose, h, sizeof(h), hipMemcpyHostToDevice, s);
  (void)hipStreamSynchronize(s);
  Se3Inputs in{pose, pose + 9, pose + 12, pose + 21, nullptr, nullptr, 0.f, false};
  launch_accum<true, false, false>(V, RV, in, cols * rows, Se3Out{scratch}, s);
  hipLaunchKernelGGL(k_final_tree_op, dim3(1), dim3(SOLVE_BLOCK), 0, s, (const float*)scratch, SE3_ACCS, op_groups(cols * rows), out29_dev);
}
void rgb_residual_op(const RgbResidualArgs& a, const int16_t* dIdx, const int16_t* dIdy, const float* lastDepth,
                     const float* nextDepth, const uint8_t* lastImage, const uint8_t* nextImage, void* corres, int cols,
                     int rows, int* out2_dev, hipStream_t s) {
  ResidualView V{dIdx, dIdy, lastDepth, nextDepth, lastImage, nextImage, (DataTerm*)corres, cols, rows, a.minScale, a.maxDepthDelta};
  float* params;
  (void)hipMalloc((void**)&params, 12 * sizeof(float));
  float h[12];
  for (int i = 0; i < 9; ++i) h[i] = a.krkinv[i];
  for (int i = 0; i < 3; ++i) h[9 + i] = a.kt[i];
  (void)hipMemcpyAsync(params, h, sizeof(h), hipMemcpyHostToDevice, s);
  (void)hipMemsetAsync(out2_dev, 0, 2 * sizeof(int), s);
  hipLaunchKernelGGL(k_rgb_residual_op, dim3(ceil_div(cols * rows, REDUCE_BLOCK)), dim3(REDUCE_BLOCK), 0, s, V, (const float*)params,
                     (const float*)(params + 9), out2_dev);
  (void)hipStreamSynchronize(s);
  (void)hipFree(params);
}
void rgb_step_op(const void* corres, float sigma, const float* cloud, float fx, float fy, const int16_t* dIdx, const int16_t* dIdy,
                 float sobelScale, int cols, int rows, float* scratch, float* out29_dev, hipStream_t s) {
  IcpView IV{};
  RgbView V{corres, nullptr, cloud, dIdx, dIdy, cols, rows, Intr{fx, fy, 0, 0}, sobelScale};
  Se3Inputs in{nullptr, nullptr, nullptr, nullptr, nullptr, nullptr, sigma, false};
  launch_accum<false, true, false>(IV, V, in, cols * rows, Se3Out{scratch}, s);
  hipLaunchKernelGGL(k_final_tree_op, dim3(1), dim3(SOLVE_BLOCK), 0, s, (const float*)scratch, SE3_ACCS, op_groups(cols * rows), out29_dev);
}
void so3_step_op(const So3Args& a, const uint8_t* lastImage, const uint8_t* nextImage, int cols, int rows, float* scratch, float* out11_dev,
                 hipStream_t s) {
  hipLaunchKernelGGL(k_so3_op, dim3(so3_grid(cols * rows)), dim3(SO3_BLOCK), 0, s, lastImage, nextImage, cols, rows, a, scratch);
  hipLaunchKernelGGL(k_final_tree_op, dim3(1), dim3(SOLVE_BLOCK), 0, s, (const float*)scratch, SO3_ACCS, op_groups(cols * rows), out11_dev);
}

namespace {
template <bool SPLIT_TAIL>
__global__ void __launch_bounds__(128) k_gn_update_probe(TrackState* st, const float* __restrict__ sums, const StepArgs A) {
  __shared__ efs::SolveScratch S;
  __shared__ float sums_s[2 * SE3_ACCS];
  const int t = threadIdx.x, wave = t >> 6;
  const GNState* prev = &st->gn[0];
  GNState* next = &st->gn[1];
  efs::SolvePrefetch PF{};
  if (t < 64) PF = efs::solve_prefetch(st, prev, &st->rgb_slots[0][0][0]);
  if (t < 2 * SE3_ACCS) sums_s[t] = sums[t];
  __syncthreads();
  if (t < 64) solve_step_wave<SPLIT_TAIL>(st, prev, next, true, sums_s, A, S, PF, true);
  __syncthreads();
  if (SPLIT_TAIL && S.tail_pending) {
    if (wave == 0) efs::gn_tail_pose(S, next, true);
    else if (wave == 1) efs::gn_tail_krk(A.knext, S, next, true);
    __syncthreads();
  }
}
__global__ void k_track_end_tail_probe(TrackState* st, const float* __restrict__ pose12, bool rgb, float weightMultiplier, double* traj) {
  if (threadIdx.x != 0) return;
  track_end_tail(st, pose12, pose12 + 9, rgb, weightMultiplier, traj, 0);
}
}

int gn_update_op(const GnUpdateProbe& p, GNState* next_host, double* lastA36, double* lastb6, float* stats4) {
  TrackState* h = new TrackState();
  h->gn[0] = p.prev;
  for (int i = 0; i < 9; ++i) h->Rprev[i] = p.Rprev[i];
  for (int i = 0; i < 3; ++i) h->tprev[i] = p.tprev[i];
  for (int l = 0; l < RGB_SLOTS; ++l) {
    h->rgb_slots[0][l][0] = p.count / RGB_SLOTS + (l < p.count % RGB_SLOTS ? 1 : 0);
    h->rgb_slots[0][l][1] = p.sigma / RGB_SLOTS + (l < p.sigma % RGB_SLOTS ? 1 : 0);
  }
  for (int i = 0; i < 36; ++i) h->lastA[i] = lastA36[i];
  for (int i = 0; i < 6; ++i) h->lastb[i] = lastb6[i];
  h->lastICPError = stats4[0]; h->lastICPCount = stats4[1]; h->lastRGBError = stats4[2]; h->lastRGBCount = stats4[3];
  StepArgs A{true, false, p.icp, p.rgb, p.rgbOnly, p.icpWeight, p.knext, p.level_changes, 1};
  TrackState* st = nullptr;
  float* sums = nullptr;
  hipError_t e = hipMalloc((void**)&st, sizeof(TrackState));
  if (e == hipSuccess) e = hipMalloc((void**)&sums, sizeof(p.sums));
  if (e == hipSuccess) e = hipMemcpy(st, h, sizeof(TrackState), hipMemcpyHostToDevice);
  if (e == hipSuccess) e = hipMemcpy(sums, p.sums, sizeof(p.sums), hipMemcpyHostToDevice);
  if (e == hipSuccess) {
    if (p.split_tail) hipLaunchKernelGGL(k_gn_update_probe<true>, dim3(1), dim3(128), 0, 0, st, (const float*)sums, A);
    else hipLaunchKernelGGL(k_gn_update_probe<false>, dim3(1), dim3(64), 0, 0, st, (const float*)sums, A);
    e = hipGetLastError();
  }
  if (e == hipSuccess) e = hipMemcpy(h, st, sizeof(TrackState), hipMemcpyDeviceToHost);
  if (st) (void)hipFree(st);
  if (sums) (void)hipFree(sums);
  if (e == hipSuccess) {
    *next_host = h->gn[1];
    for (int i = 0; i < 36; ++i) lastA36[i] = h->lastA[i];
    for (int i = 0; i < 6; ++i) lastb6[i] = h->lastb[i];
    stats4[0] = h->lastICPError; stats4[1] = h->lastICPCount; stats4[2] = h->lastRGBError; stats4[3] = h->lastRGBCount;
  }
  delete h;
  return (int)e;
}

int track_end_tail_op(TrackState* st_host, const float* pose12, bool rgb, float weightMultiplier, double* logged16) {
  TrackState* st = nullptr;
  float* pose = nullptr;
  double* traj = nullptr;
  hipError_t e = hipMalloc((void**)&st, sizeof(TrackState));
  if (e == hipSuccess) e = hipMalloc((void**)&pose, 12 * sizeof(float));
  if (e == hipSuccess) e = hipMalloc((void**)&traj, 16 * sizeof(double));
  if (e == hipSuccess) e = hipMemcpy(st, st_host, sizeof(TrackState), hipMemcpyHostToDevice);
  if (e == hipSuccess) e = hipMemcpy(pose, pose12, 12 * sizeof(float), hipMemcpyHostToDevice);
  if (e == hipSuccess) {
    hipLaunchKernelGGL(k_track_end_tail_probe, dim3(1), dim3(64), 0, 0, st, (const float*)pose, rgb, weightMultiplier, traj);
    e = hipGetLastError();
  }
  if (e == hipSuccess) e = hipMemcpy(st_host, st, sizeof(TrackState), hipMemcpyDeviceToHost);
  if (e == hipSuccess) e = hipMemcpy(logged16, traj, 16 * sizeof(double), hipMemcpyDeviceToHost);
  if (st) (void)hipFree(st);
  if (pose) (void)hipFree(pose);
  if (traj) (void)hipFree(traj);
  return (int)e;
}
```

### elasticfusion_amd/csrc/ef_track_kernels.hip

```cpp
#include "ef_device.hpp"
#include "ef_linalg_dev.hpp"
#include "ef_solve_dev.hpp"
#include <stddef.h>
#include <initializer_list>
#include <mutex>
#include <type_traits>
#include <hip/hip_ext.h>
#include "ef_track.hpp"

using namespace ef;

namespace eft {

namespace {

constexpr int TILE_X = 64, TILE_Y = 4;

inline dim3 tile_grid(int cols, int rows) { return dim3((cols + TILE_X - 1) / TILE_X, (rows + TILE_Y - 1) / TILE_Y); }
inline dim3 tile_block() { return dim3(TILE_X, TILE_Y); }


__device__ __forceinline__ void pyr_down_u16_px(const uint16_t* __restrict__ src, int scols, int srows, uint16_t* __restrict__ dst, int x, int y) {
  const int dcols = scols / 2;
  const int D = 5;
// ... 1491 lines not shown
  EF_ASTAMP(0);
  f32x4 c[3];
#pragma unroll
  for (int q = 0; q < 3; ++q) c[q] = f32x4{0.f, 0.f, 0.f, 0.f};
  if (HAS_ICP && !rgb_wave) accum_quads<CH, true, PACKED>(IV, RV, in, gbase, N, K, 0, 0, false, c);
  if (HAS_RGB && rgb_wave) accum_quads<CH, false, PACKED>(IV, RV, in, gbase, N, K, slot_a, slot_b, with_slots, c);
  EF_ASTAMP(3);
  if (half == 1) {
#pragma unroll
    for (int q = 0; q < 3; ++q) {
      xch[wl][tix][q * 4 + 0][lane] = c[q].x; xch[wl][tix][q * 4 + 1][lane] = c[q].y;
      xch[wl][tix][q * 4 + 2][lane] = c[q].z; xch[wl][tix][q * 4 + 3][lane] = c[q].w;
    }
  }
  __syncthreads();
  EF_ASTAMP(4);
  float r[12];
  if (half == 0) {
#pragma unroll
    for (int q = 0; q < 3; ++q) {
      r[q * 4 + 0] = c[q].x + xch[wl][tix][q * 4 + 0][lane]; r[q * 4 + 1] = c[q].y + xch[wl][tix][q * 4 + 1][lane];
      r[q * 4 + 2] = c[q].z + xch[wl][tix][q * 4 + 2][lane]; r[q * 4 + 3] = c[q].w + xch[wl][tix][q * 4 + 3][lane];
    }
#pragma unroll
    for (int i = 0; i < 12; ++i) {
      r[i] += down32(r[i]);
      r[i] += down16(r[i]);
      r[i] += row_down<8>(r[i]);
      r[i] += row_down<4>(r[i]);
    }
    if (wl == 1 && v == 0) {
#pragma unroll
      for (int i = 0; i < 12; ++i) pair[tix][i][j] = r[i];
    }
  }
  __syncthreads();
  if (half == 0 && wl == 0 && v == 0) {
    float* dst = out.pairs + (size_t)tix * SE3_ACCS * SE3_PAIRS + wg;
#pragma unroll
    for (int q = 0; q < 3; ++q)
#pragma unroll
      for (int i = 0; i < 4; ++i) {
        const int a = quad_member(q, i, j);
        if (a >= 0) dst[(size_t)a * SE3_PAIRS] = r[q * 4 + i] + pair[tix][q * 4 + i][j];
      }
  }
  EF_ASTAMP(5);
}

#ifdef EF_FAST_ORDER
#include "ef_track_fast.inc"
#endif

template <int BLOCK, int NA, bool COHERENT>
__device__ __forceinline__ void final_tree(const float* partials, float* bs, float* out) {
  static_assert((NA * VWARPS) % 64 == 0 && BLOCK % 64 == 0, "whole waves");
  constexpr int TOTAL = NA * VWARPS, PASSES = (TOTAL + BLOCK - 1) / BLOCK;
  const int t = threadIdx.x;
  float v[PASSES];
#pragma unroll
  for (int j = 0; j < PASSES; ++j) {
    const int idx = t + j * BLOCK, q = idx < TOTAL ? idx : 0;
    v[j] = COHERENT ? __hip_atomic_load(partials + q, __ATOMIC_RELAXED, __HIP_MEMORY_SCOPE_AGENT) : partials[q];
  }
#pragma unroll
  for (int j = 0; j < PASSES; ++j) {
    const int idx = t + j * BLOCK;
    float x = v[j];
    x += __shfl_down(x, 4, 8);
    x += __shfl_down(x, 2, 8);
    x += __shfl_down(x, 1, 8);
    if (idx < TOTAL && (idx & 7) == 0) bs[idx >> 3] = x;
  }
  __syncthreads();
  for (int idx = t; idx < NA * 64; idx += BLOCK) {
    float x = bs[idx];
#pragma unroll
    for (int off = 16; off > 0; off >>= 1) x += __shfl_down(x, off, 32);
    const float w1 = __shfl(x, 32, 64);
    if ((idx & 63) == 0) out[idx >> 6] = x + w1;
  }
  __syncthreads();
}

template <typename T>
__host__ __device__ inline void unpack29(const float* h, T* A, T* b) {
  int shift = 0;
  for (int i = 0; i < 6; ++i)
    for (int j = i; j < 7; ++j) {
      const float value = h[shift++];
      if (j == 6) b[i] = (T)value;
      else A[j * 6 + i] = A[i * 6 + j] = (T)value;
    }
}

__device__ inline void compute_krk(const double* resultRt, Intr k, float* krkinv, float* kt) {
  double Rt[16];
  efl::m4_affine_inverse(resultRt, Rt);
  double R[9], K[9] = {k.fx, 0, k.cx, 0, k.fy, k.cy, 0, 0, 1}, Kinv[9], KR[9], KRK[9];
  for (int r = 0; r < 3; ++r)
    for (int c = 0; c < 3; ++c) R[r * 3 + c] = Rt[r * 4 + c];
  efl::m3_inverse<double>(K, Kinv);
  efl::m3_mul(K, R, KR);
  efl::m3_mul(KR, Kinv, KRK);
  for (int i = 0; i < 9; ++i) krkinv[i] = (float)KRK[i];
  const double tv[3] = {Rt[3], Rt[7], Rt[11]};
  double Kt[3];
  efl::m3_mulv(K, tv, Kt);
  for (int i = 0; i < 3; ++i) kt[i] = (float)Kt[i];
}

__device__ inline void so3_matrices(const double* resultR, Intr k, float* mats27) {
  double K[9] = {k.fx, 0, k.cx, 0, k.fy, k.cy, 0, 0, 1}, Kinv[9], KR[9], H[9];
  efl::m3_inverse<double>(K, Kinv);
  efl::m3_mul(K, resultR, KR);
  efl::m3_mul(KR, Kinv, H);
  for (int i = 0; i < 9; ++i) { mats27[i] = (float)H[i]; mats27[9 + i] = (float)Kinv[i]; mats27[18 + i] = (float)KR[i]; }
}

__global__ void k_track_begin(TrackState* st, bool so3, Intr kso3, Intr kfirst) {
  if (threadIdx.x != 0) return;
  double R[9];
  efl::quat_to_mat<double>(st->q, R);
  GNState& g = st->gn[0];
  for (int i = 0; i < 9; ++i) st->Rprev[i] = g.Rcurr[i] = (float)R[i];
  for (int i = 0; i < 3; ++i) st->tprev[i] = g.tcurr[i] = (float)st->t[i];
  efl::m3_inverse<float>(st->Rprev, st->Rprev_inv);
  for (int i = 0; i < 4; ++i) st->q_prev[i] = st->q[i];
  for (int i = 0; i < 3; ++i) st->t_prev[i] = st->t[i];
  efl::m4_identity(g.resultRt);
  for (int i = 0; i < RGB_SLOTS; ++i) st->rgb_slots[0][i][0] = st->rgb_slots[0][i][1] = st->rgb_slots[1][i][0] = st->rgb_slots[1][i][1] = 0;
  g.rgb_broken = 0;
  g.lastRGBErrorLevel = 3.402823466e+38f;
  st->call_seq += 1u;
  st->so3_iterations = 0;
  st->dbg_clock[11] = ~0ull; st->dbg_clock[12] = 0;
  st->so3_ticket = 0;
  st->dense_count = 0;
  if (so3) {
    efl::m3_identity(st->so3_resultR);
    efl::m3_identity(st->so3_lastResultR);
    for (int i = 0; i < 9; ++i) st->so3_R_lr[i] = (i % 4 == 0) ? 1.f : 0.f;
    st->so3_lastError = 3.402823466e+38f / 2;
    st->so3_lastCount = 3.402823466e+38f / 2;
    st->so3_done = 0;
    so3_matrices(st->so3_resultR, kso3, st->so3_mats);
  } else {
    st->so3_done = 1;
    compute_krk(g.resultRt, kfirst, g.krkinv, g.kt);
  }
}

constexpr int SOLVE_BLOCK = 512;
template <bool SPLIT_TAIL>
__device__ __forceinline__ void solve_step_wave(TrackState* st, const GNState* prev, GNState* next, bool publish, const float* sums,
                                                const StepArgs& A, efs::SolveScratch& S, const efs::SolvePrefetch& PF, bool stats) {
  const int lane = threadIdx.x & 63;
  int sigma = PF.slot_b, rgbSize = PF.slot_a;
#pragma unroll
  for (int off = 32; off > 0; off >>= 1) {
    rgbSize += __shfl_down(rgbSize, off, 64);
    sigma += __shfl_down(sigma, off, 64);
  }
  rgbSize = __shfl(rgbSize, 0, 64);
  sigma = __shfl(sigma, 0, 64);
  efs::solve_prefetch_publish(PF, S);
  const float lastLevelErr = PF.lastRGBErrorLevel;
  const bool broken = PF.broken != 0;
  const float rgbError = (float)(sqrt((double)sigma) / (rgbSize == 0 ? 1 : rgbSize));
  const bool brk = !broken && A.rgbOnly && rgbError > lastLevelErr;
  if (broken || brk) {
    if (lane == 0) {
      S.tail_pending = 0;
      S.broken = A.level_changes ? 0 : 1;
      if (A.level_changes) {
        compute_krk(prev->resultRt, A.knext, S.krkinv, S.kt);
      } else {
        for (int i = 0; i < 9; ++i) S.krkinv[i] = prev->krkinv[i];
        for (int i = 0; i < 3; ++i) S.kt[i] = prev->kt[i];
      }
      for (int i = 0; i < 9; ++i) S.Rcurr[i] = prev->Rcurr[i];
      for (int i = 0; i < 3; ++i) S.tcurr[i] = prev->tcurr[i];
      if (publish) {
        for (int i = 0; i < 9; ++i) { next->Rcurr[i] = S.Rcurr[i]; next->krkinv[i] = S.krkinv[i]; }
        for (int i = 0; i < 3; ++i) { next->tcurr[i] = S.tcurr[i]; next->kt[i] = S.kt[i]; }
        for (int i = 0; i < 16; ++i) next->resultRt[i] = prev->resultRt[i];
        next->rgb_broken = S.broken;
        next->lastRGBErrorLevel = A.level_changes ? 3.402823466e+38f : lastLevelErr;
      }
    }
    efs::wave_sync();
    return;
  }
  if (lane == 0) {
    S.broken = 0;
    if (publish) {
      next->rgb_broken = 0;
      next->lastRGBErrorLevel = A.level_changes ? 3.402823466e+38f : rgbError;
    }
    if (stats) {
      st->lastRGBError = rgbError;
      st->lastRGBCount = (float)rgbSize;
      if (A.icp) {
        st->lastICPError = sqrtf(sums[27]) / sums[28];
        st->lastICPCount = sums[28];
      } else {
        st->lastICPError = __int_as_float(0x7fc00000);
        st->lastICPCount = 0.f;
      }
    }
  }
  EF_STAMP(st, 3);
  efs::SolveInputs in{A.icp, A.rgb, A.rgbOnly, A.icpWeight, A.knext, A.level_changes};
  efs::gauss_newton_update_wave<SPLIT_TAIL>(st, next, publish, sums, in, S, stats);
}
template <int BLOCK>
__device__ __forceinline__ void half_partials_tree(const float* __restrict__ pairs, bool icp, bool rgb, float* sums_s) {
  static_assert(BLOCK % 64 == 0, "one wavefront per accumulator");
  const int t = threadIdx.x;
  const int na = (icp ? SE3_ACCS : 0) + (rgb ? SE3_ACCS : 0);
  constexpr int PASSES = (2 * SE3_ACCS * 64 + BLOCK - 1) / BLOCK;
  unsigned long long v[PASSES];
#pragma unroll
  for (int q = 0; q < PASSES; ++q) {
    const int idx = t + q * BLOCK;
    v[q] = idx < na * 64 ? __hip_atomic_load((const unsigned long long*)pairs + (size_t)idx * 2, __ATOMIC_RELAXED, __HIP_MEMORY_SCOPE_AGENT) : 0ull;
  }
#pragma unroll
  for (int q = 0; q < PASSES; ++q) {
    const int idx = t + q * BLOCK;
    float x = __uint_as_float((unsigned)v[q]) + __uint_as_float((unsigned)(v[q] >> 32));
#pragma unroll
    for (int off = 16; off > 0; off >>= 1) x += __shfl_down(x, off, 32);
    const float w1 = __shfl(x, 32, 64);
    if (idx < na * 64 && (idx & 63) == 0) sums_s[(icp ? 0 : SE3_ACCS) + (idx >> 6)] = x + w1;
  }
}
template <int BLOCK, bool COHERENT>
__device__ __forceinline__ void pair_partials_tree(const float* __restrict__ pairs, bool icp, bool rgb, float* sums_s) {
  static_assert(BLOCK % 64 == 0, "one wavefront per accumulator");
  const int t = threadIdx.x;
  const int na = (icp ? SE3_ACCS : 0) + (rgb ? SE3_ACCS : 0);
  constexpr int PASSES = (2 * SE3_ACCS * 64 + BLOCK - 1) / BLOCK;
  float4 v[PASSES];
#pragma unroll
  for (int q = 0; q < PASSES; ++q) {
    const int idx = t + q * BLOCK;
    if (COHERENT) {
      unsigned long long lo = 0ull, hi = 0ull;
      if (idx < na * 64) {
        const unsigned long long* src = (const unsigned long long*)pairs + (size_t)idx * 2;
        lo = __hip_atomic_load(src, __ATOMIC_RELAXED, __HIP_MEMORY_SCOPE_AGENT);
        hi = __hip_atomic_load(src + 1, __ATOMIC_RELAXED, __HIP_MEMORY_SCOPE_AGENT);
      }
      v[q] = make_float4(__uint_as_float((unsigned)lo), __uint_as_float((unsigned)(lo >> 32)), __uint_as_float((unsigned)hi),
                         __uint_as_float((unsigned)(hi >> 32)));
    } else {
      v[q] = idx < na * 64 ? ((const float4*)pairs)[idx] : make_float4(0.f, 0.f, 0.f, 0.f);
    }
  }
#pragma unroll
  for (int q = 0; q < PASSES; ++q) {
    const int idx = t + q * BLOCK;
    float x = (v[q].x + v[q].z) + (v[q].y + v[q].w);
#pragma unroll
    for (int off = 16; off > 0; off >>= 1) x += __shfl_down(x, off, 32);
    const float w1 = __shfl(x, 32, 64);
    if (idx < na * 64 && (idx & 63) == 0) sums_s[(icp ? 0 : SE3_ACCS) + (idx >> 6)] = x + w1;
  }
}

template <int BLOCK>
__device__ __forceinline__ void head_sums(const float* __restrict__ pairs, int ng, bool icp, bool rgb, float* sums_s) {
#ifdef EF_FAST_ORDER
  fast_tree<BLOCK, false>(pairs, ng, (icp ? SE3_ACCS : 0) + (rgb ? SE3_ACCS : 0), sums_s + (icp ? 0 : SE3_ACCS));
#else
  if (ng == 1) {
    const int na = (icp ? SE3_ACCS : 0) + (rgb ? SE3_ACCS : 0);
    if ((int)threadIdx.x < na) sums_s[(icp ? 0 : SE3_ACCS) + threadIdx.x] = pairs[(size_t)threadIdx.x * 256];
  } else {
    pair_partials_tree<BLOCK>(pairs, icp, rgb, sums_s);
  }
#endif
}

__device__ inline void publish_pose(TrackState* st) {
  efl::SE3 T;
  for (int i = 0; i < 4; ++i) T.q[i] = st->q[i];
  for (int i = 0; i < 3; ++i) T.t[i] = st->t[i];
  efl::se3_inverse_matrix_f(T, st->T_cw);
  efl::se3_castf_matrix(T, st->pose_f);
  double R[9];
  efl::quat_to_mat<double>(T.q, R);
  for (int i = 0; i < 9; ++i) st->R_wc_f[i] = (float)R[i];
  for (int i = 0; i < 3; ++i) st->t_wc_f[i] = (float)T.t[i];
}
__device__ inline void compute_weighting(TrackState* st, float weightMultiplier) {
  efl::SE3 T, Tp;
  for (int i = 0; i < 4; ++i) { T.q[i] = st->q[i]; Tp.q[i] = st->q_prev[i]; }
  for (int i = 0; i < 3; ++i) { T.t[i] = st->t[i]; Tp.t[i] = st->t_prev[i]; }
  const efl::SE3 Tcp = efl::se3_mul(efl::se3_inverse(T), Tp);
  const double tn = sqrt(Tcp.t[0] * Tcp.t[0] + Tcp.t[1] * Tcp.t[1] + Tcp.t[2] * Tcp.t[2]);
  const double ln = efl::se3_log_norm(Tcp);
  float weighting = (float)(tn > ln ? tn : ln);
  const float largest = 0.01f, minWeight = 0.5f;
  if (weighting > largest) weighting = largest;
  const float w = 1.0f - (weighting / largest);
  st->weighting = (w > minWeight ? w : minWeight) * weightMultiplier;
}
__device__ inline void log_pose(const TrackState* st, double* traj, int slot) {
  if (!traj) return;
  efl::SE3 T;
  for (int i = 0; i < 4; ++i) T.q[i] = st->q[i];
  for (int i = 0; i < 3; ++i) T.t[i] = st->t[i];
  efl::se3_matrix(T, traj + (size_t)slot * 16);
}
__device__ __forceinline__ void track_end_tail(TrackState* st, const float* Rc_in, const float* tc_in, bool rgb, float weightMultiplier, double* traj, int slot);
__global__ void __launch_bounds__(REDUCE_BLOCK) k_track_end(TrackState* st, const GNState* __restrict__ prev, GNState* next,
                                                             const float* __restrict__ pairs, const int* __restrict__ slots_prev, const StepArgs A,
                                                             bool rgb, float weightMultiplier, double* traj, int slot, const unsigned* abort_word,
                                                             unsigned* abort_report) {
  __shared__ efs::SolveScratch S;
  __shared__ float sums_s[2 * SE3_ACCS];
  const int t = threadIdx.x;
  if (A.has_head) {
    efs::SolvePrefetch PF{};
    if (t < 64) PF = efs::solve_prefetch(st, prev, slots_prev);
    head_sums<REDUCE_BLOCK>(pairs, A.ng, A.icp, A.rgb, sums_s);
    __syncthreads();
    if (t < 64) solve_step_wave(st, prev, next, true, sums_s, A, S, PF, true);
    __syncthreads();
  } else if (t == 0) {
    for (int i = 0; i < 9; ++i) S.Rcurr[i] = prev->Rcurr[i];
    for (int i = 0; i < 3; ++i) S.tcurr[i] = prev->tcurr[i];
  }
  if (t != 0) return;
  track_end_tail(st, S.Rcurr, S.tcurr, rgb, weightMultiplier, traj, slot);
  if (abort_report) {
    const unsigned v = __hip_atomic_load(abort_word, __ATOMIC_RELAXED, __HIP_MEMORY_SCOPE_AGENT);
    if (v) __hip_atomic_store(abort_report, v, __ATOMIC_RELAXED, __HIP_MEMORY_SCOPE_SYSTEM);
  }
}
__device__ __forceinline__ void track_end_tail(TrackState* st, const float* Rc_in, const float* tc_in, bool rgb, float weightMultiplier, double* traj, int slot) {
  float Rcurr[9], tcurr[3];
  for (int i = 0; i < 9; ++i) Rcurr[i] = Rc_in[i];
  for (int i = 0; i < 3; ++i) tcurr[i] = tc_in[i];
  if (rgb) {
    const float d0 = tcurr[0] - st->tprev[0], d1 = tcurr[1] - st->tprev[1], d2 = tcurr[2] - st->tprev[2];
    if ((double)sqrtf(d0 * d0 + d1 * d1 + d2 * d2) > 0.3) {
      for (int i = 0; i < 9; ++i) Rcurr[i] = st->Rprev[i];
      for (int i = 0; i < 3; ++i) tcurr[i] = st->tprev[i];
    }
  }
  double Rc[9], Rp[9];
  for (int i = 0; i < 9; ++i) Rc[i] = (double)Rcurr[i];
  efl::polar3(Rc, Rp);
  efl::SE3 T;
  efl::se3_set_rotation(T, Rp);
  for (int i = 0; i < 4; ++i) st->q[i] = T.q[i];
  for (int i = 0; i < 3; ++i) st->t[i] = (double)tcurr[i];
  publish_pose(st);
  compute_weighting(st, weightMultiplier);
  log_pose(st, traj, slot);
}
__global__ void k_pose_injected(TrackState* st, efl::SE3 T, bool save_prev, float weightMultiplier, bool with_weighting, double* traj,
                                int slot) {
  if (threadIdx.x != 0) return;
// ... 782 lines not shown
```

### elasticfusion_amd/csrc/ef_track_ref_persistent.inc

```
constexpr int RT_KC = FT_BLOCK / 64;
__device__ __forceinline__ int rt_column(int wg) { return (wg & 7) * (FT_WGS >> 3) + (wg >> 3); }
__device__ __forceinline__ int rt_vwarp(int col, int wl) { return 8 * (col >> 2) + (col & 3) + 4 * wl; }
__device__ __forceinline__ int rt_pixel(int col, int idx) { return (idx >> 6) * VTHREADS + rt_vwarp(col, (idx >> 5) & 1) * 32 + (idx & 31); }

__device__ __forceinline__ float warp32_pair_tree(float x) {
  x += down16(x);
  x += row_down<8>(x);
  x += row_down<4>(x);
  x += row_down<2>(x);
  x += row_down<1>(x);
  return x + down32(x);
}
__device__ __forceinline__ int wave_sum_lane0(int v) {
  float x = __int_as_float(v);
  auto add = [](float a, float b) { return __int_as_float(__float_as_int(a) + __float_as_int(b)); };
  x = add(x, down32(x));
  x = add(x, down16(x));
  x = add(x, row_down<8>(x));
  x = add(x, row_down<4>(x));
  x = add(x, row_down<2>(x));
  x = add(x, row_down<1>(x));
  return __float_as_int(x);
}
__device__ __forceinline__ float rt_tree(float s0, float s1, float s2, float s3) {
// ... 275 lines not shown
  (void)IV; (void)P;
  const int S = (K + 3) >> 2, lane = threadIdx.x & 63;
#pragma unroll 1
  for (int s = 0; s < S; ++s) {
    const uint32_t* p = slots + (size_t)s * RT_RGB_WORDS * 64 + lane;
    const uint32_t gxy = p[128], corr = p[192];
    const f3 pt{__uint_as_float(p[320]), __uint_as_float(p[384]), __uint_as_float(p[256])};
    const float invz = __uint_as_float(p[448]);
    float rows[8] = {0.f, 0.f, 0.f, 0.f, 0.f, 0.f, 0.f, 0.f};
    if (corr & 0x80000000u) {
      const int gx = (int)(int16_t)(gxy & 0xFFFFu), gy = (int)(int16_t)(gxy >> 16);
      const float diff = (float)((int)((corr >> 22) & 0x1FFu) - 255);
      float w = sigma + fabsf(diff);
      w = w > 1.19209290E-07F ? 1.0f / w : 1.0f;
      if (sigma == -1) w = 1;
      rows[6] = -w * diff;
      const float dI_dx_val = w * RV.sobelScale * gx;
      const float dI_dy_val = w * RV.sobelScale * gy;
      const float v0 = dI_dx_val * RV.k.fx * invz;
      const float v1 = dI_dy_val * RV.k.fy * invz;
      const float v2 = -(v0 * pt.x + v1 * pt.y) * invz;
      rows[0] = v0; rows[1] = v1; rows[2] = v2;
      rows[3] = -pt.z * v1 + pt.y * v2;
      rows[4] = pt.z * v0 - pt.x * v2;
      rows[5] = -pt.y * v0 + pt.x * v1;
      rows[7] = 1.f;
    }
    rt_rows_to_sums(rows, s, K, c);
  }
}
#define EF_RT_RGB_PREPARE 1

template <int NT>
__device__ __forceinline__ void rt_column_trees(const f32x4 (&c)[3], float* xch , float* pairx , float (&r)[12]) {
  const int t = threadIdx.x, lane = t & 63, wave = t >> 6;
  const int v = lane >> 2, j = lane & 3;
  const int tix = wave >> 2, rem = wave & 3, wl = rem >> 1, half = rem & 1;
  const bool active = wave < 4 * NT;
  float* xw = xch + (size_t)((active ? wl : 0) * NT + (active ? tix : 0)) * 12 * 64;
  if (active && half == 1) {
#pragma unroll
    for (int q = 0; q < 3; ++q) {
      xw[(q * 4 + 0) * 64 + lane] = c[q].x; xw[(q * 4 + 1) * 64 + lane] = c[q].y;
      xw[(q * 4 + 2) * 64 + lane] = c[q].z; xw[(q * 4 + 3) * 64 + lane] = c[q].w;
    }
  }
  __syncthreads();
  if (active && half == 0) {
#pragma unroll
    for (int q = 0; q < 3; ++q) {
      r[q * 4 + 0] = c[q].x + xw[(q * 4 + 0) * 64 + lane]; r[q * 4 + 1] = c[q].y + xw[(q * 4 + 1) * 64 + lane];
      r[q * 4 + 2] = c[q].z + xw[(q * 4 + 2) * 64 + lane]; r[q * 4 + 3] = c[q].w + xw[(q * 4 + 3) * 64 + lane];
    }
#pragma unroll
    for (int i = 0; i < 12; ++i) {
      r[i] += down32(r[i]);
      r[i] += down16(r[i]);
      r[i] += row_down<8>(r[i]);
      r[i] += row_down<4>(r[i]);
    }
    if (wl == 1 && v == 0) {
#pragma unroll
      for (int i = 0; i < 12; ++i) pairx[((size_t)tix * 12 + i) * 4 + j] = r[i];
    }
  }
  __syncthreads();
  if (active && half == 0 && wl == 0 && v == 0) {
#pragma unroll
    for (int i = 0; i < 12; ++i) r[i] = r[i] + pairx[((size_t)tix * 12 + i) * 4 + j];
  }
}
template <bool HAS_ICP, bool HAS_RGB, bool PAIRS = true, typename Hook>
__device__ __forceinline__ void rt_accumulate(const IcpView& IV, const RgbView& RV, const IcpPose& P, int col, int N, int K,
                                              float* xch , float* pairx , float (&r)[12], Hook wait_sigma,
                                              const float* icp_slots = nullptr) {
  constexpr int NT = (HAS_ICP && HAS_RGB) ? 2 : 1;
  const int wave = threadIdx.x >> 6;
  const int tix = wave >> 2, rem = wave & 3, wl = rem >> 1, half = rem & 1;
  const bool active = wave < 4 * NT;
  const bool rgb_wave = HAS_RGB && (!HAS_ICP || tix == 1);
  f32x4 c[3];
#pragma unroll
  for (int q = 0; q < 3; ++q) c[q] = f32x4{0.f, 0.f, 0.f, 0.f};
  if (active) {
    const int gbase = rt_vwarp(col, wl) * 32 + half * 16;
    if (HAS_ICP && !rgb_wave) {
      if (icp_slots) rt_icp_resident(IV, RV, P, icp_slots + (size_t)rem * ((K + 3) >> 2) * 6 * 64, gbase, N, K, c);
      else accum_quads_rolled<true, RtNoWait, PAIRS>(IV, RV, P, gbase, N, K, c, RtNoWait{0.f});
    }
    if (HAS_RGB && rgb_wave) accum_quads_rolled<false, Hook, PAIRS>(IV, RV, P, gbase, N, K, c, wait_sigma);
  }
  rt_column_trees<NT>(c, xch, pairx, r);
}
__device__ __forceinline__ void rt_so3_accumulate(const uint8_t* __restrict__ lastImage, const uint8_t* __restrict__ nextImage, int cols, int rows,
                                                  const m33& IB, const m33& KI, const m33& KR, int col, float* lds_rows ,
                                                  float (&z)[SO3_ACCS]) {
  const int t = threadIdx.x, lane = t & 63, N = cols * rows;
  const int K = (N + VTHREADS - 1) / VTHREADS;
  const int gl = rt_vwarp(col, lane >> 5) * 32 + (lane & 31);
  const int nk = gl < N ? (N - gl + VTHREADS - 1) / VTHREADS : 0;
#pragma unroll
  for (int i = 0; i < SO3_ACCS; ++i) z[i] = 0.f;
  for (int k0 = 0; k0 < K; k0 += RT_KC) {
    const int kc = min(RT_KC, K - k0);
    {
      const int k = t >> 6;
      if (k < kc) {
        const int p = rt_pixel(col, (k0 + k) * 64 + lane);
        float row[4] = {0.f, 0.f, 0.f, 0.f};
        float found = 0.f;
        if (p < N && so3_row(lastImage, nextImage, cols, rows, IB, KI, KR, p, row)) found = 1.f;
        float* rr = lds_rows + (size_t)k * 5 * 64 + lane;
        rr[0] = row[0]; rr[64] = row[1]; rr[128] = row[2]; rr[192] = row[3]; rr[256] = found;
      }
    }
    __syncthreads();
    if (t < 64) {
      const int kend = min(kc, nk - k0);
      for (int k = 0; k < kend; ++k) {
        const float* rr = lds_rows + (size_t)k * 5 * 64 + lane;
        const float r0 = rr[0], r1 = rr[64], r2 = rr[128], r3 = rr[192], f = rr[256];
        z[0] = EF_FMA(r0, r0, z[0]); z[1] = EF_FMA(r0, r1, z[1]); z[2] = EF_FMA(r0, r2, z[2]); z[3] = EF_FMA(r0, r3, z[3]);
        z[4] = EF_FMA(r1, r1, z[4]); z[5] = EF_FMA(r1, r2, z[5]); z[6] = EF_FMA(r1, r3, z[6]);
        z[7] = EF_FMA(r2, r2, z[7]); z[8] = EF_FMA(r2, r3, z[8]);
        z[9] = EF_FMA(r3, r3, z[9]);
        z[10] += f;
      }
    }
    __syncthreads();
  }
  if (t < 64) {
#pragma unroll
    for (int i = 0; i < SO3_ACCS; ++i) {
      z[i] = warp32_pair_tree(z[i]);
    }
  }
}

template <bool HAS_ICP, bool HAS_RGB>
__global__ void __launch_bounds__(FT_BLOCK) k_track_ref(const FtArgs A, TrackState* st) {
  constexpr int NT = (HAS_ICP && HAS_RGB) ? 2 : 1;
  constexpr int NA = NT * SE3_ACCS;
  __shared__ GNState gs[2];
  __shared__ efs::SolveScratch S;
  __shared__ float sums_s[2 * SE3_ACCS];
  __shared__ float bg[24];
  __shared__ float xch[2 * 2 * 12 * 64];
  __shared__ float pairx[2 * 12 * 4];
  __shared__ float lds_rows[RT_KC * 5 * 64];
  __shared__ float red[SO3_ACCS];
  __shared__ So3Loop Z;
  __shared__ int ired[2 * FT_BLOCK / 64];
  __shared__ int tot_s[2];
  __shared__ unsigned seen_a[2];
  __shared__ int dead_s;
  __shared__ unsigned mode_s;
  __shared__ int wsum[4][2];
  __shared__ unsigned wtag[4];
  extern __shared__ __attribute__((aligned(16))) float rt_res[];
  const int t = threadIdx.x, lane = t & 63, wave = t >> 6, wg = blockIdx.x;
  const int col = rt_column(wg);
  constexpr int RGB_W0 = HAS_ICP ? 4 : 0;
#ifdef EF_STAGE_CLOCKS
  unsigned long long clk_last2 = 0;
#define FT_CLK2(i) do { if (wg == 0 && t == RGB_W0 * 64) { const unsigned long long now_ = wall_clock64(); (void)__hip_atomic_fetch_add(&Y->clk[i], now_ - clk_last2, __ATOMIC_RELAXED, __HIP_MEMORY_SCOPE_AGENT); clk_last2 = now_; } } while (0)
#else
#define FT_CLK2(i) do { } while (0)
#endif
  unsigned long long* G1 = (unsigned long long*)(A.partials + FT_G1_OFF);
  unsigned long long* G2 = (unsigned long long*)(A.partials + FT_G2R_OFF);
  unsigned long long* GA = (unsigned long long*)(A.partials + FT_GAR_OFF);
  const unsigned long long* G2_mine = G2 + (size_t)(blockIdx.x & (FT_REPL - 1)) * FT_REPL_STRIDE;
  const unsigned long long* GA_mine = GA + (size_t)(blockIdx.x & (FT_REPL_A - 1)) * FT_REPL_STRIDE;
  FtSync* Y = (FtSync*)(A.partials + FT_SY_OFF);
#ifdef EF_STAGE_CLOCKS
  unsigned long long clk_last = wall_clock64();
  const unsigned long long clk_start = clk_last;
#endif
  if (A.empty_model_flag && *A.empty_model_flag != A.empty_model_value) {
    if (wg != 0 || t != 0) return;
    double R[9];
    efl::quat_to_mat<double>(st->q, R);
    GNState& o = st->gn[A.out_cur];
    float Rp[9], Rpi[9];
    for (int i = 0; i < 9; ++i) Rp[i] = o.Rcurr[i] = (float)R[i];
    for (int i = 0; i < 3; ++i) o.tcurr[i] = (float)st->t[i];
    efl::m3_inverse<float>(Rp, Rpi);
    efl::m4_identity(o.resultRt);
    o.rgb_broken = 0;
    o.lastRGBErrorLevel = 0.f;
    compute_krk(o.resultRt, A.L[0].k, o.krkinv, o.kt);
    for (int i = 0; i < 9; ++i) { st->Rprev[i] = Rp[i]; st->Rprev_inv[i] = Rpi[i]; }
    for (int i = 0; i < 3; ++i) st->tprev[i] = o.tcurr[i];
    for (int i = 0; i < 4; ++i) st->q_prev[i] = st->q[i];
    for (int i = 0; i < 3; ++i) st->t_prev[i] = st->t[i];
    for (int i = 0; i < RGB_SLOTS; ++i) st->rgb_slots[0][i][0] = st->rgb_slots[0][i][1] = st->rgb_slots[1][i][0] = st->rgb_slots[1][i][1] = 0;
    st->call_seq += 1u;
    st->so3_iterations = 0;
    st->so3_ticket = 0;
    st->so3_done = 1;
    st->dense_count = 0;
    float* P = A.partials + FT_P_OFF;
    for (int a = 0; a < NA; ++a) P[(size_t)a * 256] = 0.f;
    return;
  }
  if (t == 64) ft_put(&Y->arrive[wg], 1u, A.epoch);
  if (wg == 0 && wave == 7) {
    bool ok[4] = {false, false, false, false};
    bool all = false;
    for (int spin = 0; spin < FT_ADMIT_SPIN && !all; ++spin) {
#pragma unroll
      for (int i = 0; i < 4; ++i)
        if (!ok[i]) ok[i] = (unsigned)(ft_get(&Y->arrive[64 * i + lane]) >> 32) == A.epoch;
      all = __all(ok[0] && ok[1] && ok[2] && ok[3]);
      if (!all && spin > 8) __builtin_amdgcn_s_sleep(2);
    }
    if (!all) {
      static_assert(sizeof(FtArgs) % 4 == 0, "copied dword by dword");
      typedef const __attribute__((address_space(4))) unsigned* KWords;
      const KWords src = (KWords)__builtin_amdgcn_kernarg_segment_ptr();
      unsigned* dst = (unsigned*)&Y->args;
      for (int i = lane; i < (int)(sizeof(FtArgs) / 4); i += 64) dst[i] = src[i];
    }
    if (lane == 0 && !all) {
      __hip_atomic_fetch_add(&Y->fallbacks, 1u, __ATOMIC_RELAXED, __HIP_MEMORY_SCOPE_AGENT);
      drain_stores();
    }
    const unsigned verdict = all ? FT_MODE_PERSISTENT : FT_MODE_SERIAL;
    if (lane < FT_REPL) ft_put(G2 + (size_t)lane * FT_REPL_STRIDE + FT_MODE_WORD, verdict, A.epoch);
    if (lane == 0) ft_put(&Y->mode, verdict, A.epoch);
  }
  if (t == 128) {
    unsigned m = 0u;
    for (int spin = 0; spin < FT_SPIN; ++spin) {
      const unsigned long long g = ft_get(G2_mine + FT_MODE_WORD);
      if ((unsigned)(g >> 32) == A.epoch) { m = (unsigned)g; break; }
      if (spin > 8) __builtin_amdgcn_s_sleep(1);
    }
    mode_s = m;
  }
  if (t == 0) {
    dead_s = (int)__hip_atomic_load(&Y->abort, __ATOMIC_RELAXED, __HIP_MEMORY_SCOPE_AGENT);
    seen_a[0] = 0u;
    seen_a[1] = 0u;
    tot_s[0] = tot_s[1] = 0;
    wtag[0] = wtag[1] = wtag[2] = wtag[3] = 0u;
    double R[9];
    efl::quat_to_mat<double>(st->q, R);
    GNState& g = gs[0];
    for (int i = 0; i < 9; ++i) bg[i] = g.Rcurr[i] = (float)R[i];
    for (int i = 0; i < 3; ++i) bg[9 + i] = g.tcurr[i] = (float)st->t[i];
    efl::m3_inverse<float>(bg, bg + 12);
    efl::m4_identity(g.resultRt);
    g.rgb_broken = 0;
    g.lastRGBErrorLevel = 3.402823466e+38f;
    if (!A.so3) compute_krk(g.resultRt, A.kfirst, g.krkinv, g.kt);
  }
  __syncthreads();
  FT_CLK(0);
  if (dead_s) return;
  if (mode_s == 0u) {
    if (t == 0) __hip_atomic_store(&Y->abort, 1u, __ATOMIC_RELAXED, __HIP_MEMORY_SCOPE_AGENT);
    return;
  }
  if (mode_s == FT_MODE_SERIAL) return;
  if (wg == 0 && t == 0) {
    for (int i = 0; i < 9; ++i) { st->Rprev[i] = bg[i]; st->Rprev_inv[i] = bg[12 + i]; }
    for (int i = 0; i < 3; ++i) st->tprev[i] = bg[9 + i];
    for (int i = 0; i < 4; ++i) st->q_prev[i] = st->q[i];
    for (int i = 0; i < 3; ++i) st->t_prev[i] = st->t[i];
    for (int i = 0; i < RGB_SLOTS; ++i) st->rgb_slots[0][i][0] = st->rgb_slots[0][i][1] = st->rgb_slots[1][i][0] = st->rgb_slots[1][i][1] = 0;
    st->call_seq += 1u;
    st->so3_iterations = 0;
    st->so3_ticket = 0;
    st->so3_done = 1;
    st->dense_count = 0;
  }
  unsigned epoch = A.epoch;
  int cur = 0;
  if (A.so3) {
    if (t == 0) {
      efl::m3_identity(Z.resR);
      efl::m3_identity(Z.lastResR);
      for (int i = 0; i < 9; ++i) Z.R_lr[i] = (i % 4 == 0) ? 1.f : 0.f;
      Z.lastError = 3.402823466e+38f / 2;
      Z.lastCount = 3.402823466e+38f / 2;
      Z.done = 0;
      so3_matrices(Z.resR, A.kso3, Z.mats);
    }
    __syncthreads();
    for (int it = 0; it < 10; ++it, ++epoch) {
      {
        const m33 IB = m33_load(Z.mats), KI = m33_load(Z.mats + 9), KR = m33_load(Z.mats + 18);
        float z[SO3_ACCS];
        rt_so3_accumulate(A.so3_last, A.so3_next, A.so3_cols, A.so3_rows, IB, KI, KR, col, lds_rows, z);
        if (t == 0) {
#pragma unroll
          for (int i = 0; i < SO3_ACCS; ++i) ft_put(G1 + (size_t)i * 256 + ft_slot(col), __float_as_uint(z[i]), epoch);
        }
      }
      FT_CLK(1);
      if (wave == 1 && wg < SO3_ACCS) rt_reduce_publish(G1, G2, wg, epoch, &dead_s, Y, nullptr);
      if (wave == 0) {
        float v;
        ft_poll_totals(G2_mine, SO3_ACCS, epoch, &dead_s, Y, v);
        if (lane < SO3_ACCS) red[lane] = v;
      }
      __syncthreads();
      FT_CLK(2);
      if (t == 0) Z.done = so3_update(Z, red, it, A.kso3, A.kfirst, gs[0]) ? 1 : 0;
      __syncthreads();
      FT_CLK(4);
      FT_COUNT(20);
      if (Z.done) { ++epoch; break; }
    }
    if (wg == 0 && t == 0) {
      st->lastSO3Error = Z.err;
      st->lastSO3Count = Z.cnt;
      st->so3_iterations = Z.iterations;
    }
  }
  for (int it = 0; it < A.n_iter; ++it) {
    const int lvl = ft_level_of(A.levels, it);
#ifdef EF_STAGE_CLOCKS
    const unsigned long long clk_iter = wall_clock64();
#endif
    const PtLevel Lv = ft_load_level((FtArgsK)__builtin_amdgcn_kernarg_segment_ptr(), lvl);
    const int cols = Lv.cols, rows = Lv.rows, N = cols * rows;
    const int K = (N + VTHREADS - 1) / VTHREADS;
    const bool last = it == A.n_iter - 1;
    const int NS = (K + 3) >> 2;
    const int res = rt_res_mode(HAS_ICP, HAS_RGB, NS, A.res_bytes);
    float* const icp_res = rt_res;
    uint32_t* const rgb_res = (uint32_t*)(rt_res + (HAS_ICP ? (size_t)NS * (RT_ICP_STEP_BYTES / 4) : 0));
    const IcpView IV{Lv.vmap_curr, Lv.nmap_curr, Lv.vmap_g_prev, Lv.nmap_g_prev, cols, rows, Lv.k, A.distThres, A.angleThres, A.dist2Max, A.sine2Max};
    const RgbView RV{Lv.corres, Lv.lastDepth, nullptr, Lv.dIdx, Lv.dIdy, cols, rows, Lv.k, 1.0f / 8.0f};
    if (res && (it == 0 || lvl != ft_level_of(A.levels, it - 1))) {
      const int nfill = wave == 0 ? 0 : (wave == 7 ? 2 : 1);
#pragma unroll 1
      for (int f = 0; f < nfill; ++f) {
        const int w = f == 0 ? wave : 0, rem = w & 3;
        const int gbase = rt_vwarp(col, rem >> 1) * 32 + (rem & 1) * 16;
        if (HAS_ICP && w < 4) rt_fill_icp(IV, RV, icp_res + (size_t)rem * NS * 6 * 64, gbase, N, K);
        if (HAS_RGB && res == 2 && w >= RGB_W0 && w < RGB_W0 + 4) rt_fill_rgb(Lv, rgb_res + (size_t)rem * NS * RT_RGB_WORDS * 64, gbase, N, K);
      }
      if (it == 0) __syncthreads();
    }
    if (it > 0) {
      StepArgs H{true, false, HAS_ICP, HAS_RGB, false, A.icpWeight, Lv.k, lvl != ft_level_of(A.levels, it - 1), it};
      if (t < 64) {
        efs::SolvePrefetch PF{};
        const GNState& gp = gs[cur];
        PF.rt = gp.resultRt[lane & 15];
        PF.pose = bg[lane < 12 ? lane : 0];
        PF.slot_a = (HAS_RGB && lane == 0) ? tot_s[0] : 0;
        PF.slot_b = (HAS_RGB && lane == 0) ? tot_s[1] : 0;
        PF.lastRGBErrorLevel = gp.lastRGBErrorLevel;
        PF.broken = gp.rgb_broken;
        solve_step_wave<true>(st, &gs[cur], &gs[cur ^ 1], true, sums_s, H, S, PF, false);
      }
      __syncthreads();
      if (S.tail_pending) {
        if (wave == 0) efs::gn_tail_pose(S, &gs[cur ^ 1], true);
        else if (wave == 1) efs::gn_tail_krk(H.knext, S, &gs[cur ^ 1], true);
        __syncthreads();
      }
      FT_CLK(6);
#ifdef EF_STAGE_CLOCKS
      if (wg == 0 && t == 0) {
        const unsigned long long* c = st->dbg_clock;
        FT_ADD(3, c[4] - c[3]); FT_ADD(5, c[5] - c[4]); FT_ADD(18, c[6] - c[5]); FT_ADD(19, c[7] - c[6]); FT_ADD(23, c[8] - c[7]);
      }
#endif
      cur ^= 1;
    }
    const GNState& G = gs[cur];
    const unsigned epoch_a = epoch;
    if (HAS_RGB && res == 2) {
      ++epoch;
      FT_CLK(7);
    } else if (HAS_RGB) {
      int cnt = 0, sq = 0;
      const m33 Km = m33_load(G.krkinv);
      const f3 kt{G.kt[0], G.kt[1], G.kt[2]};
      const int npx = 64 * K;
      if (npx > FT_BLOCK) {
#pragma unroll 1
        for (int e0 = t; e0 < npx; e0 += 3 * FT_BLOCK) {
          int qs[3], nis[3], gi[3], u0s[3], v0s[3], lis[3];
          uint8_t m[3];
          float d1s[3], td1[3], d0s[3];
#pragma unroll
          for (int e = 0; e < 3; ++e) {
            const int idx = e0 + e * FT_BLOCK;
            const int q = rt_pixel(col, idx);
            const bool in = idx < npx && q < N;
            const int qq = in ? q : N - 1;
            qs[e] = q;
            m[e] = in ? Lv.mask[qq] : (uint8_t)0;
            d1s[e] = Lv.nextDepth[qq];
            nis[e] = Lv.nextImage[qq];
          }
#pragma unroll
          for (int e = 0; e < 3; ++e) {
            const int q = qs[e];
            const int y = q / cols, x = q - y * cols;
            const float d1 = d1s[e];
            td1[e] = (float)(d1 * (Km.r[2].x * x + Km.r[2].y * y + Km.r[2].z) + kt.z);
            u0s[e] = f2i_rn((d1 * (Km.r[0].x * x + Km.r[0].y * y + Km.r[0].z) + kt.x) / td1[e]);
            v0s[e] = f2i_rn((d1 * (Km.r[1].x * x + Km.r[1].y * y + Km.r[1].z) + kt.y) / td1[e]);
            gi[e] = (m[e] && u0s[e] >= 0 && v0s[e] >= 0 && u0s[e] < cols && v0s[e] < rows) ? v0s[e] * cols + u0s[e] : -1;
            d0s[e] = 0.f;
            lis[e] = 0;
            if (gi[e] >= 0) { d0s[e] = Lv.lastDepth[gi[e]]; lis[e] = Lv.lastImage[gi[e]]; }
          }
#pragma unroll
          for (int e = 0; e < 3; ++e) {
            if (!m[e]) continue;
            uint32_t packed = 0u;
            if (gi[e] >= 0 && d0s[e] > 0 && fabsf(td1[e] - d0s[e]) <= 0.07f  && lis[e] != 0) {
              const int idiff = nis[e] - lis[e];
              packed = pack_corres(u0s[e], v0s[e], idiff);
              cnt += 1;
              sq += idiff * idiff;
            }
            Lv.corres[qs[e]] = packed;
          }
        }
      } else {
        const int q = rt_pixel(col, t);
        const bool in = t < npx && q < N;
        const int qq = in ? q : N - 1;
        const uint8_t mk = Lv.mask[qq];
        const float d1 = Lv.nextDepth[qq];
        const int ni = Lv.nextImage[qq];
        if (in && mk) {
          const int y = q / cols, x = q - y * cols;
          const float td = (float)(d1 * (Km.r[2].x * x + Km.r[2].y * y + Km.r[2].z) + kt.z);
          const int u0 = f2i_rn((d1 * (Km.r[0].x * x + Km.r[0].y * y + Km.r[0].z) + kt.x) / td);
          const int v0 = f2i_rn((d1 * (Km.r[1].x * x + Km.r[1].y * y + Km.r[1].z) + kt.y) / td);
          uint32_t packed = 0u;
          if (u0 >= 0 && v0 >= 0 && u0 < cols && v0 < rows) {
            const int gi1 = v0 * cols + u0;
            const float d0 = Lv.lastDepth[gi1];
            const int li = Lv.lastImage[gi1];
            if (d0 > 0 && fabsf(td - d0) <= 0.07f  && li != 0) {
              const int idiff = ni - li;
              packed = pack_corres(u0, v0, idiff);
              cnt += 1;
              sq += idiff * idiff;
            }
          }
          Lv.corres[q] = packed;
        }
      }
      cnt = wave_sum_lane0(cnt);
      sq = wave_sum_lane0(sq);
      if (lane == 0) { ired[wave * 2] = cnt; ired[wave * 2 + 1] = sq; }
      __syncthreads();
      if (t == 0) {
        int sa = 0, sb = 0;
        for (int w = 0; w < FT_BLOCK / 64; ++w) { sa += ired[w * 2]; sb += ired[w * 2 + 1]; }
#pragma unroll
        for (int c = 0; c < FT_REPL_A; ++c) {
          ft_put(GA + (size_t)c * FT_REPL_STRIDE + 2 * col, (unsigned)sa, epoch_a);
          ft_put(GA + (size_t)c * FT_REPL_STRIDE + 2 * col + 1, (unsigned)sb, epoch_a);
        }
      }
      ++epoch;
      FT_CLK(7);
    }
    const unsigned epoch_b = epoch++;
    IcpPose P{};
    if (HAS_ICP) {
      P.Rcurr = m33_load(G.Rcurr);
      P.tcurr = {G.tcurr[0], G.tcurr[1], G.tcurr[2]};
      P.Rprev_inv = m33_load(bg + 12);
      P.tprev = {bg[9], bg[10], bg[11]};
      if (res) {
        auto u1 = [](float x) { return __uint_as_float(__builtin_amdgcn_readfirstlane(__float_as_uint(x))); };
        auto u3 = [&](f3 a) { return f3{u1(a.x), u1(a.y), u1(a.z)}; };
        P.Rcurr = m33{{u3(P.Rcurr.r[0]), u3(P.Rcurr.r[1]), u3(P.Rcurr.r[2])}};
        P.tcurr = u3(P.tcurr);
        P.Rprev_inv = m33{{u3(P.Rprev_inv.r[0]), u3(P.Rprev_inv.r[1]), u3(P.Rprev_inv.r[2])}};
        P.tprev = u3(P.tprev);
      }
    }
    auto wait_sigma = [&]() -> float {
      const bool leader = (wave & 3) == 0;
      if (leader) {
        int sa, sb;
        const bool ok = ft_sweep_records(GA_mine, epoch_a, &dead_s, Y, sa, sb);
        sa = wave_sum_lane0(sa);
        sb = wave_sum_lane0(sb);
        if (lane == 0) {
          tot_s[0] = sa;
          tot_s[1] = sb;
          __hip_atomic_store(&seen_a[1], ok ? 0u : 1u, __ATOMIC_RELAXED, __HIP_MEMORY_SCOPE_WORKGROUP);
          __hip_atomic_store(&seen_a[0], epoch_a, __ATOMIC_RELEASE, __HIP_MEMORY_SCOPE_WORKGROUP);
        }
      } else if (lane == 0) {
        int spins = 0;
        while (__hip_atomic_load(&seen_a[0], __ATOMIC_ACQUIRE, __HIP_MEMORY_SCOPE_WORKGROUP) != epoch_a && ++spins < 64 * FT_SPIN) __builtin_amdgcn_s_sleep(1);
      }
      efs::wave_sync();
      const int rgbSize = __builtin_amdgcn_readfirstlane(__hip_atomic_load(&tot_s[0], __ATOMIC_RELAXED, __HIP_MEMORY_SCOPE_WORKGROUP));
      const int sqsum = __builtin_amdgcn_readfirstlane(__hip_atomic_load(&tot_s[1], __ATOMIC_RELAXED, __HIP_MEMORY_SCOPE_WORKGROUP));
      return sigma_from_sums(sqsum, rgbSize, false);
    };
    float r[12];
    if (res == 2) {
      const int rem = wave & 3;
      const int gbase = rt_vwarp(col, rem >> 1) * 32 + (rem & 1) * 16;
      f32x4 c[3];
#pragma unroll
      for (int q = 0; q < 3; ++q) c[q] = f32x4{0.f, 0.f, 0.f, 0.f};
      if (HAS_ICP && wave < 4) {
// ... 413 lines not shown
```

### include/ef_hip.h

```cpp
#ifndef EF_HIP_H_
#define EF_HIP_H_
#include <stddef.h>
#include <stdint.h>
#ifdef __cplusplus
extern "C" {
#endif

#define EF_OK 0
#define EF_EINVAL (-1)
#define EF_EHIP (-2)
#define EF_ENOMEM (-3)
#define EF_ESTATE (-4)
#define EF_ECAPACITY (-5)

typedef struct ef_ctx ef_ctx;

typedef struct ef_config {
  int width, height;
  float fx, fy, cx, cy;
  int time_delta;
  float confidence;
  float depth_cut;
  float icp_weight;
  int fast_odom;
// ... 429 lines not shown
typedef struct ef_plane_result {
  uint32_t nodes, planes, on_rows, off_rows, count_after;
} ef_plane_result;
int ef_default_plane_params(ef_ctx* ctx, ef_plane_params* params);
int ef_map_planes(ef_ctx* ctx, const ef_plane_params* params, const ef_map_selection* among_or_null, uint32_t* plane_or_null, uint32_t max_rows,
                  ef_plane_model* models_or_null, ef_plane_result* result_or_null);
int ef_map_planes_dev(ef_ctx* ctx, const ef_plane_params* params, const ef_map_selection* among_or_null, uint32_t* plane_dev_or_null,
                      uint32_t max_rows, ef_plane_model* models_dev_or_null, ef_plane_result* result_dev_or_null);
int ef_map_planes_select(ef_ctx* ctx, const ef_plane_params* params, const ef_map_selection* among_or_null, int what, int which, uint32_t* rows,
                         uint32_t max_rows, uint32_t* count, ef_plane_model* models_or_null, ef_plane_result* result_or_null);
int ef_map_planes_select_dev(ef_ctx* ctx, const ef_plane_params* params, const ef_map_selection* among_or_null, int what, int which,
                             uint32_t* rows_dev, uint32_t max_rows, uint32_t* count_dev, ef_plane_model* models_dev_or_null,
                             ef_plane_result* result_dev_or_null);
int ef_map_remove_planes(ef_ctx* ctx, const ef_plane_params* params, const ef_map_selection* among_or_null, int which,
                         ef_plane_model* models_or_null, ef_plane_result* result);

enum ef_image {
  EF_IMG_DEPTH_FILTERED = 0,
  EF_IMG_DEPTH_METRIC,
  EF_IMG_DEPTH_METRIC_FILTERED,
  EF_IMG_PREDICT_IMAGE,
  EF_IMG_PREDICT_VERTEX,
  EF_IMG_PREDICT_NORMAL,
  EF_IMG_PREDICT_TIME,
  EF_IMG_FILL_IMAGE,
  EF_IMG_FILL_VERTEX,
  EF_IMG_FILL_NORMAL,
  EF_IMG_INDEX,
  EF_IMG_VERT_CONF,
  EF_IMG_COLOR_TIME,
  EF_IMG_NORM_RAD,
  EF_IMG_OLD_IMAGE,
  EF_IMG_OLD_VERTEX,
  EF_IMG_OLD_NORMAL,
  EF_IMG_OLD_TIME
};
int ef_get_image(ef_ctx* ctx, int which, void* host_dst, size_t bytes);
int ef_get_image_resized(ef_ctx* ctx, int which, int factor, void* host_dst, size_t bytes);
int ef_get_tracker_buffer(ef_ctx* ctx, int which, int level, void* host_dst, size_t bytes);
int ef_get_tracker_buffer_of(ef_ctx* ctx, int tracker, int which, int level, void* host_dst, size_t bytes);

typedef struct ef_timing { const char* name; float ms; } ef_timing;
int ef_enable_timing(ef_ctx* ctx, int on);
int ef_get_timings(ef_ctx* ctx, ef_timing* out, int max, int* n);

typedef struct ef_kernel_time {
  const char* name; float avg_us; int launches; double bytes_per_launch; double bytes_per_launch_survey;
} ef_kernel_time;
int ef_kernel_timing(ef_ctx* ctx, int every_n_frames);
int ef_get_kernel_timing(ef_ctx* ctx, ef_kernel_time* out);
int ef_get_splat_timing(ef_ctx* ctx, ef_kernel_time* out);
int ef_get_tracker_timing(ef_ctx* ctx, ef_kernel_time* out);

int ef_get_tracker_fallbacks(ef_ctx* ctx, int* count);
typedef struct ef_tracker_plan {
  int script, n_small, n_iter;
  unsigned long long levels;
  unsigned res_bytes, res_budget;
} ef_tracker_plan;
int ef_get_tracker_plan(ef_ctx* ctx, ef_tracker_plan* out);
int ef_debug_occupy(ef_ctx* ctx, int workgroups, int microseconds);
int ef_debug_query_lanes(ef_ctx* ctx, int lanes);
int ef_debug_inject_tracker_abort(ef_ctx* ctx);

int ef_debug_clocks(ef_ctx* ctx, unsigned long long* out16);
int ef_debug_small_clocks(ef_ctx* ctx, unsigned long long* out32);

int ef_dev_alloc(void** dev, size_t bytes);
int ef_dev_free(void* dev);
int ef_dev_upload(void* dev, const void* host, size_t bytes);
int ef_dev_download(void* host, const void* dev, size_t bytes);
int ef_dev_memset(void* dev, int value, size_t bytes);
int ef_dev_sync(void);
int ef_dev_calibrate(void* stream, float* empty_us, float* stream16mb_us);
int ef_device_count(int* n);
int ef_set_device(int device);

typedef struct ef_intr { float fx, fy, cx, cy; } ef_intr;

int ef_op_pyr_down(const uint16_t* src, int src_cols, int src_rows, uint16_t* dst, void* stream);
int ef_op_create_vmap(const ef_intr* intr, const uint16_t* depth, int cols, int rows, float depth_cutoff,
                      float* vmap, void* stream);
int ef_op_create_nmap(const float* vmap, int cols, int rows, float* nmap, void* stream);
int ef_op_transform_maps(const float* vmap_src, const float* nmap_src, int cols, int rows, const float* R9,
                         const float* t3, float* vmap_dst, float* nmap_dst, void* stream);
int ef_op_copy_maps(const float* vmap_src_f4, const float* nmap_src_f4, int cols, int rows, float* vmaps_tmp,
                    float* vmap_dst, float* nmap_dst, void* stream);
int ef_op_resize_vmap(const float* in, int src_cols, int src_rows, float* out, void* stream);
int ef_op_resize_nmap(const float* in, int src_cols, int src_rows, float* out, void* stream);
int ef_op_pyr_down_gauss_f(const float* src, int src_cols, int src_rows, float* dst, void* stream);
int ef_op_pyr_down_uchar_gauss(const uint8_t* src, int src_cols, int src_rows, uint8_t* dst, void* stream);
int ef_op_vertices_to_depth(const float* vmaps_tmp, int cols, int rows, float cutoff, float* dst, void* stream);
int ef_op_image_bgr_to_intensity(const uint8_t* rgba, int cols, int rows, uint8_t* dst, void* stream);
int ef_op_compute_derivative_images(const uint8_t* src, int cols, int rows, int16_t* dx, int16_t* dy, void* stream);
int ef_op_project_to_point_cloud(const float* depth, int cols, int rows, const ef_intr* intr_level0, int level,
                                 float* cloud_f3, void* stream);
int ef_op_icp_step(const float* Rcurr9, const float* tcurr3, const float* vmap_curr, const float* nmap_curr,
                   const float* Rprev_inv9, const float* tprev3, const ef_intr* intr, const float* vmap_g_prev,
                   const float* nmap_g_prev, float dist_thres, float angle_thres, int cols, int rows,
                   float* A_host36, float* b_host6, float* residual_host2, void* stream);
int ef_op_compute_rgb_residual(float min_scale, const int16_t* dIdx, const int16_t* dIdy, const float* last_depth,
                               const float* next_depth, const uint8_t* last_image, const uint8_t* next_image,
                               void* corres_img, float max_depth_delta, const float* kt3, const float* krkinv9,
                               int cols, int rows, int* sigma_sum_host, int* count_host, void* stream);
int ef_op_rgb_step(const void* corres_img, float sigma, const float* cloud_f3, float fx, float fy,
                   const int16_t* dIdx, const int16_t* dIdy, float sobel_scale, int cols, int rows,
                   float* A_host36, float* b_host6, void* stream);
int ef_op_so3_step(const uint8_t* last_image, const uint8_t* next_image, const float* image_basis9,
                   const float* kinv9, const float* krlr9, int cols, int rows, float* A_host9, float* b_host3,
                   float* residual_host2, void* stream);

typedef struct ef_model_maps_op {
  int cols, rows;
  const float *pred_vertex, *pred_normal, *fill_vertex, *fill_normal;
  const uint8_t *pred_image, *fill_image;
  float R[9], t[3];
  float max_depth_rgb;
  int camera_frame, force_fill_image, tally;
  unsigned dense_count;
  int dense_samples;
  float* vmap[3];
  float* nmap[3];
  float* depth0;
  uint8_t* last0;
  int joint;
  const uint16_t* raw;
  const uint8_t* rgb3;
  float depth_cut;
  uint16_t* filtered;
  float* metric;
  float* metric_filtered;
  uint8_t* next0;
} ef_model_maps_op;
int ef_op_model_maps(const ef_model_maps_op* args, unsigned* dense_count_left, void* stream);
int ef_op_sobel_mask(const uint8_t* const* next_image3, const float* const* next_depth3, int cols, int rows, int16_t* const* dIdx3,
                     int16_t* const* dIdy3, uint8_t* const* mask3, uint32_t* const* corres3, void* stream);

enum ef_linalg_op {
  EF_LINALG_LDLT6 = 0,
  EF_LINALG_LDLT3F,
  EF_LINALG_POLAR3,
  EF_LINALG_RODRIGUES,
  EF_LINALG_SE3_INVERSE,
  EF_LINALG_SE3_LOG_NORM,
  EF_LINALG_SCALAR,
  EF_LINALG_LDLT6_WAVE,
  EF_LINALG_LDLT6_EVERY_LANE,
  EF_LINALG_MAT_TO_QUAT,
  EF_LINALG_SE3_MUL,
  EF_LINALG_SE3_CASTF,
  EF_LINALG_SE3_INVERSE_F,
  EF_LINALG_M4_AFFINE_INVERSE,
  EF_LINALG_LDLT_PIVOTS,
  EF_LINALG_LU_INVERSE6
};
int ef_op_linalg(int which, const double* in_host, int n_in, double* out_host, int n_out);

typedef struct ef_gn_state {
  float Rcurr[9], tcurr[3];
  double resultRt[16];
  float krkinv[9], kt[3];
  float lastRGBErrorLevel;
  int rgb_broken;
} ef_gn_state;
typedef struct ef_gn_update_args {
  float sums[58];
  ef_gn_state prev;
  float Rprev[9], tprev[3];
  int count, sigma;
  int icp, rgb, rgb_only;
  float icp_weight;
  ef_intr knext;
  int level_changes;
  int split_tail;
} ef_gn_update_args;
int ef_op_gn_update(const ef_gn_update_args* in, ef_gn_state* next, double* lastA36, double* lastb6, float* stats4);
typedef struct ef_track_end_out {
  double q[4], t[3];
  double logged[16];
  float T_cw[16], pose_f[16], R_wc_f[9], t_wc_f[3];
  float weighting;
} ef_track_end_out;
int ef_op_track_end_tail(const float* Rcurr9, const float* tcurr3, const float* Rprev9, const float* tprev3, const double* q_prev4,
                         const double* t_prev3, int rgb, float weight_multiplier, ef_track_end_out* out);

typedef struct ef_cam { int cols, rows; float fx, fy, cx, cy; } ef_cam;

int ef_op_filter_depth(const uint16_t* raw, int cols, int rows, float max_d, uint16_t* filtered, void* stream);
int ef_op_metricise_depth(const uint16_t* in, int cols, int rows, float max_d, float* out, void* stream);
int ef_op_seed_map(const ef_cam* cam, const uint8_t* rgb, const float* depth_metric, const float* depth_metric_filtered,
                   int time, float max_depth, float* surfels_aos, uint32_t* count_host, void* stream);
int ef_op_predict_indices(const ef_cam* cam, const double* T_wc16, int time, const float* surfels_aos, uint32_t count,
                          float max_depth, int time_delta, uint32_t* index_map, float* vert_conf, float* color_time,
                          float* norm_rad, void* stream);
int ef_op_combined_predict(const ef_cam* cam, const double* T_wc16, const float* surfels_aos, uint32_t count,
                           float max_depth, float conf_threshold, int time, int max_time, int time_delta,
                           uint8_t* image_rgba, float* vertex, float* normal, uint16_t* time_map, void* stream);
int ef_op_synthesize_depth(const ef_cam* cam, const double* T_wc16, const float* surfels_aos, uint32_t count,
                           float max_depth, float conf_threshold, int time, int max_time, int time_delta,
                           float* depth, void* stream);
int ef_op_fill_in(const ef_cam* cam, const uint8_t* image_rgba, const float* vertex, const float* normal,
                  const uint16_t* depth_filtered, const uint8_t* rgb, int passthrough, int passthrough_image,
                  uint8_t* fill_image, float* fill_vertex, float* fill_normal, void* stream);
int ef_op_dense_enough(const ef_cam* cam, const uint8_t* image_rgba, int* dense_host, void* stream);
int ef_op_fuse(const ef_cam* cam, const double* T_wc16, int time, const uint8_t* rgb, const float* depth_metric,
               const float* depth_metric_filtered, const uint32_t* index_map, const float* vert_conf,
               const float* color_time, const float* norm_rad, float max_depth, float weighting, float* surfels_aos,
               uint32_t count, float* new_unstable_aos, uint32_t* new_count_host, void* stream);
int ef_op_clean(const ef_cam* cam, const double* T_wc16, int time, const uint32_t* index_map, const float* vert_conf,
                const float* color_time, const float* norm_rad, float conf_threshold, int time_delta, float max_depth,
                const float* surfels_aos, uint32_t count, const float* new_unstable_aos, uint32_t new_count,
                float* surfels_out_aos, uint32_t* out_count_host, void* stream);
int ef_op_clean_deform(const ef_cam* cam, const double* T_wc16, int time, const uint32_t* index_map, const float* vert_conf,
                       const float* color_time, const float* norm_rad, float conf_threshold, int time_delta, float max_depth,
                       const float* surfels_aos, uint32_t count, const float* new_unstable_aos, uint32_t new_count,
                       const float* graph, int nodes, const float* depth, int is_fern, float* surfels_out_aos,
                       uint32_t* out_count_host, void* stream);

#ifdef __cplusplus
}
#endif
#endif
```

Baseline: 2165.

## Run GN solve step in place with per-entry cofactor inverse and offloaded RGB state

The persistent tracking kernel's Gauss-Newton step now reads the previous pose and Rt straight from shared GN state, with no per-lane prefetch copy or shuffle reduction. The precomputed lane-to-accumulator member table comes from a shared byte array. A second wave stages the intrinsics matrix and writes the RGB error state in parallel. The 3x3 inverse is computed per lane from a single cofactor rather than a full inverse per lane. This shortens the serial solve path between iterations, at the cost of more template variants and shared memory, plus a new probe path for testing.

```diff
diff --git a/elasticfusion_amd/api.py b/elasticfusion_amd/api.py
--- a/elasticfusion_amd/api.py
+++ b/elasticfusion_amd/api.py
@@ -1697,7 +1697,7 @@
         return out.to_array(np.float32, (n.value, 12))
 
     LINALG = dict(ldlt6=0, ldlt3f=1, polar3=2, rodrigues=3, se3_inverse=4, se3_log_norm=5, scalar=6, ldlt6_wave=7, ldlt6_every_lane=8,
-                  mat_to_quat=9, se3_mul=10, se3_castf=11, se3_inverse_f=12, m4_affine_inverse=13, ldlt_pivots=14, lu_inverse6=15)
+                  mat_to_quat=9, se3_mul=10, se3_castf=11, se3_inverse_f=12, m4_affine_inverse=13, ldlt_pivots=14, lu_inverse6=15, m3_inverse_lanes=16)
 
     @staticmethod
     def linalg(which, vec, n_out):
diff --git a/elasticfusion_amd/csrc/ef_host_ops.inc b/elasticfusion_amd/csrc/ef_host_ops.inc
--- a/elasticfusion_amd/csrc/ef_host_ops.inc
+++ b/elasticfusion_amd/csrc/ef_host_ops.inc
@@ -228,6 +228,16 @@
 }
 namespace {
 __global__ void k_linalg_probe(int which, const double* __restrict__ in, double* __restrict__ out) {
+  if (which == EF_LINALG_M3_INVERSE_LANES) {
+    __shared__ double m4[12];
+    const int lane = threadIdx.x;
+    if (lane < 9) m4[(lane / 3) * 4 + lane % 3] = in[lane];
+    efs::wave_sync();
+    const double v = efs::m3_inverse_entry(m4, lane < 9 ? lane : 0);
+    if (lane < 9) out[lane] = v;
+    if (lane == 0) efl::m3_inverse<double>(in, out + 9);
+    return;
+  }
   if (which == EF_LINALG_LDLT6_WAVE || which == EF_LINALG_LDLT6_EVERY_LANE) {
     __shared__ efs::SolveScratch S;
     const int lane = threadIdx.x;
@@ -286,7 +296,7 @@
 }
 extern "C" {
 int ef_op_linalg(int which, const double* in, int n_in, double* out, int n_out) {
-  if (!in || !out || n_in <= 0 || n_out <= 0 || n_in > 64 || n_out > 64 || which < 0 || which > EF_LINALG_LU_INVERSE6) return EF_EINVAL;
+  if (!in || !out || n_in <= 0 || n_out <= 0 || n_in > 64 || n_out > 64 || which < 0 || which > EF_LINALG_M3_INVERSE_LANES) return EF_EINVAL;
   double* d;
   if (hipMalloc((void**)&d, 128 * sizeof(double)) != hipSuccess) return EF_ENOMEM;
   (void)hipMemset(d, 0, 128 * sizeof(double));
@@ -300,7 +310,7 @@
 
 static_assert(sizeof(ef_gn_state) == sizeof(eft::GNState), "ef_gn_state is eft::GNState");
 int ef_op_gn_update(const ef_gn_update_args* in, ef_gn_state* next, double* lastA36, double* lastb6, float* stats4) {
-  if (!in || !next || !lastA36 || !lastb6 || !stats4 || !(in->icp || in->rgb)) return EF_EINVAL;
+  if (!in || !next || !lastA36 || !lastb6 || !stats4 || !(in->icp || in->rgb) || in->split_tail < 0 || in->split_tail > 2) return EF_EINVAL;
   eft::GnUpdateProbe p;
   memcpy(p.sums, in->sums, sizeof(p.sums));
   memcpy(&p.prev, &in->prev, sizeof(p.prev));
@@ -310,7 +320,7 @@
   p.icpWeight = in->icp_weight;
   p.knext = eft::Intr{in->knext.fx, in->knext.fy, in->knext.cx, in->knext.cy};
   p.level_changes = in->level_changes != 0;
-  p.split_tail = in->split_tail != 0;
+  p.form = in->split_tail;
   const hipError_t e = (hipError_t)eft::gn_update_op(p, (eft::GNState*)next, lastA36, lastb6, stats4);
   if (e != hipSuccess) { g_create_error = hipGetErrorString(e); return e == hipErrorOutOfMemory ? EF_ENOMEM : EF_EHIP; }
   return EF_OK;
diff --git a/elasticfusion_amd/csrc/ef_solve_dev.hpp b/elasticfusion_amd/csrc/ef_solve_dev.hpp
--- a/elasticfusion_amd/csrc/ef_solve_dev.hpp
+++ b/elasticfusion_amd/csrc/ef_solve_dev.hpp
@@ -38,6 +38,12 @@
   float Rcurr[9], tcurr[3];
   int broken;
   int tail_pending;
+  double K4[12];
+};
+struct SolveSource {
+  const double* prevRt;
+  const float* prevPose;
+  const unsigned char* member;
 };
 struct SolvePrefetch {
   double rt;
@@ -63,10 +69,19 @@
   if (lane < 12) S.prevPose[lane] = P.pose;
 }
 
+__device__ __forceinline__ SolveSource solve_source_of(const SolveScratch& S) { return SolveSource{S.prevRt, S.prevPose, nullptr}; }
+
 __device__ __forceinline__ int se3_member_of(int i, int j) {
   const int lo = i < j ? i : j, hi = i < j ? j : i;
   const int start = lo * 7 - (lo * (lo - 1)) / 2;
   return start + (hi - lo);
+}
+
+__device__ __forceinline__ int gn_member_of_lane(int lane) {
+  const int e = lane < 36 ? lane : 0;
+  const int i = e / 6, j = e - i * 6;
+  const int bi = lane >= 36 && lane < 42 ? lane - 36 : 0;
+  return lane < 36 ? se3_member_of(i, j) : se3_member_of(bi, 6);
 }
 
 __device__ __forceinline__ void ldlt6_wave(double a, SolveScratch& S) {
@@ -133,13 +148,18 @@
   wave_sync();
 }
 
-__device__ __forceinline__ double m3_inverse_entry(const double* m, int e) {
-  double o[9];
-  efl::m3_inverse<double>(m, o);
-  double r = o[0];
-#pragma unroll
-  for (int q = 1; q < 9; ++q) r = (e == q) ? o[q] : r;
-  return r;
+__device__ __forceinline__ double m3_inverse_entry(const double* m4, int e) {
+  constexpr unsigned OPS[9] = {0x96a5u, 0xa192u, 0x5261u, 0xa486u, 0x82a0u, 0x6042u, 0x8594u, 0x9081u, 0x4150u};
+  unsigned ops = OPS[0];
+#pragma unroll
+  for (int q = 1; q < 9; ++q) ops = (e == q) ? OPS[q] : ops;
+  const double a = m4[ops & 15u], b = m4[(ops >> 4) & 15u], c = m4[(ops >> 8) & 15u], d = m4[(ops >> 12) & 15u];
+  const double c00 = m4[5] * m4[10] - m4[6] * m4[9];
+  const double c01 = m4[6] * m4[8] - m4[4] * m4[10];
+  const double c02 = m4[4] * m4[9] - m4[5] * m4[8];
+  const double det = m4[0] * c00 + m4[1] * c01 + m4[2] * c02;
+  const double id = 1.0 / det;
+  return (a * b - c * d) * id;
 }
 
 __device__ __forceinline__ constexpr int ldlt6_at(int i, int j) { return i >= j ? i * (i + 1) / 2 + j : j * (j + 1) / 2 + i; }
@@ -235,7 +255,8 @@
   bool level_changes;
 };
 
-__device__ __forceinline__ void gn_tail_pose(SolveScratch& S, eft::GNState* next, bool publish) {
+template <bool IN_PLACE = false>
+__device__ __forceinline__ void gn_tail_pose(SolveScratch& S, eft::GNState* next, bool publish, const float* prevPose = nullptr) {
   const int lane = threadIdx.x & 63;
   if (lane < 12) {
     float iR[9], ot[3], it[3];
@@ -247,32 +268,42 @@
     }
 #pragma unroll
     for (int r = 0; r < 3; ++r) it[r] = -(iR[r * 3] * ot[0] + iR[r * 3 + 1] * ot[1] + iR[r * 3 + 2] * ot[2]);
-    const float* Rp = S.prevPose;
+    const float* Rp = IN_PLACE ? prevPose : S.prevPose;
     if (lane < 9) {
       const int r = lane / 3, c = lane - r * 3;
       const float i0 = (float)S.Rt[c * 4], i1 = (float)S.Rt[c * 4 + 1], i2 = (float)S.Rt[c * 4 + 2];
       const float v = Rp[r * 3] * i0 + Rp[r * 3 + 1] * i1 + Rp[r * 3 + 2] * i2;
-      S.Rcurr[lane] = v;
-      if (publish) next->Rcurr[lane] = v;
+      if (!IN_PLACE) S.Rcurr[lane] = v;
+      if (IN_PLACE || publish) next->Rcurr[lane] = v;
     } else {
       const int r = lane - 9;
-      const float v = (Rp[r * 3] * it[0] + Rp[r * 3 + 1] * it[1] + Rp[r * 3 + 2] * it[2]) + S.prevPose[9 + r];
-      S.tcurr[r] = v;
-      if (publish) next->tcurr[r] = v;
-    }
-  }
-}
+      const float v = (Rp[r * 3] * it[0] + Rp[r * 3 + 1] * it[1] + Rp[r * 3 + 2] * it[2]) + Rp[9 + r];
+      if (!IN_PLACE) S.tcurr[r] = v;
+      if (IN_PLACE || publish) next->tcurr[r] = v;
+    }
+  }
+}
+__device__ __forceinline__ void gn_stage_K(const eft::Intr k, SolveScratch& S) {
+  const int lane = threadIdx.x & 63;
+  if (lane >= 16 && lane < 25) {
+    const int q = lane - 16, r = q / 3, c = q - r * 3;
+    const double v = (q == 0) ? (double)k.fx : (q == 2) ? (double)k.cx : (q == 4) ? (double)k.fy : (q == 5) ? (double)k.cy : (q == 8) ? 1.0 : 0.0;
+    S.K4[r * 4 + c] = v;
+  }
+}
+template <bool IN_PLACE = false, bool K_STAGED = false>
 __device__ __forceinline__ void gn_tail_krk(const eft::Intr knext, SolveScratch& S, eft::GNState* next, bool publish) {
   const int lane = threadIdx.x & 63;
   {
     const eft::Intr k = knext;
     const double K[9] = {k.fx, 0, k.cx, 0, k.fy, k.cy, 0, 0, 1};
+    if (!K_STAGED) {
+      gn_stage_K(knext, S);
+      wave_sync();
+    }
     const bool second = lane >= 16;
-    double m[9];
-#pragma unroll
-    for (int q = 0; q < 9; ++q) m[q] = second ? K[q] : S.Rt[(q / 3) * 4 + (q % 3)];
     const int e = second ? lane - 16 : lane;
-    const double inv = m3_inverse_entry(m, (e >= 0 && e < 9) ? e : 0);
+    const double inv = m3_inverse_entry(second ? S.K4 : S.Rt, (e >= 0 && e < 9) ? e : 0);
     if (lane < 9) S.inv[0][lane] = inv;
     else if (lane >= 16 && lane < 25) S.inv[1][lane - 16] = inv;
     wave_sync();
@@ -295,31 +326,27 @@
       double s = 0;
 #pragma unroll
       for (int kk = 0; kk < 3; ++kk) s += S.KR[r * 3 + kk] * S.inv[1][kk * 3 + c];
-      S.krkinv[lane] = (float)s;
-      if (publish) next->krkinv[lane] = (float)s;
+      if (!IN_PLACE) S.krkinv[lane] = (float)s;
+      if (IN_PLACE || publish) next->krkinv[lane] = (float)s;
     } else if (lane >= 16 && lane < 19) {
       const int r = lane - 16;
       const double t0 = -S.ti[0], t1 = -S.ti[1], t2 = -S.ti[2];
       const double k0 = (r == 0) ? K[0] : 0.0, k1 = (r == 1) ? K[4] : 0.0, k2 = (r == 0) ? K[2] : (r == 1 ? K[5] : 1.0);
       const float v = (float)(k0 * t0 + k1 * t1 + k2 * t2);
-      S.kt[r] = v;
-      if (publish) next->kt[r] = v;
-    }
-  }
-  wave_sync();
-}
-template <bool SPLIT_TAIL = false>
+      if (!IN_PLACE) S.kt[r] = v;
+      if (IN_PLACE || publish) next->kt[r] = v;
+    }
+  }
+  wave_sync();
+}
+template <bool SPLIT_TAIL = false, bool IN_PLACE = false>
 __device__ __forceinline__ void gauss_newton_update_wave(eft::TrackState* st, eft::GNState* next, bool publish, const float* sums,
-                                                         const SolveInputs in, SolveScratch& S, bool stats) {
+                                                         const SolveInputs in, SolveScratch& S, bool stats, const SolveSource src) {
+  static_assert(SPLIT_TAIL || !IN_PLACE, "the in-place step leaves its tails to the caller");
   const int lane = threadIdx.x & 63;
   double a = 0.0;
   {
-    const int e = lane < 36 ? lane : 0;
-    const int i = e / 6, j = e - i * 6;
-    const int mA = se3_member_of(i, j);
-    const int bi = lane >= 36 && lane < 42 ? lane - 36 : 0;
-    const int mb = se3_member_of(bi, 6);
-    const int m = lane < 36 ? mA : mb;
+    const int m = IN_PLACE ? (int)src.member[lane] : gn_member_of_lane(lane);
     double v;
     if (in.icp && in.rgb) {
       const double w = in.icpWeight;
@@ -376,21 +403,23 @@
     const int r = lane >> 2, c = lane & 3;
     double s = 0;
 #pragma unroll
-    for (int k = 0; k < 4; ++k) s += S.upd[r * 4 + k] * S.prevRt[k * 4 + c];
+    for (int k = 0; k < 4; ++k) s += S.upd[r * 4 + k] * src.prevRt[k * 4 + c];
     S.Rt[lane] = s;
-  }
-  wave_sync();
-  if (publish && lane < 16) next->resultRt[lane] = S.Rt[lane];
-  if (SPLIT_TAIL) {
-    if (lane == 0) S.tail_pending = 1;
-    wave_sync();
-    return;
-  }
+    if (IN_PLACE || publish) next->resultRt[lane] = s;
+  }
+  if (SPLIT_TAIL && lane == 0) S.tail_pending = 1;
+  wave_sync();
+  if (SPLIT_TAIL) return;
   gn_tail_pose(S, next, publish);
   EF_STAMP(st, 7);
   gn_tail_krk(in.knext, S, next, publish);
   wave_sync();
   EF_STAMP(st, 8);
 }
-
-}
+template <bool SPLIT_TAIL = false>
+__device__ __forceinline__ void gauss_newton_update_wave(eft::TrackState* st, eft::GNState* next, bool publish, const float* sums,
+                                                         const SolveInputs in, SolveScratch& S, bool stats) {
+  gauss_newton_update_wave<SPLIT_TAIL, false>(st, next, publish, sums, in, S, stats, solve_source_of(S));
+}
+
+}
diff --git a/elasticfusion_amd/csrc/ef_track.hpp b/elasticfusion_amd/csrc/ef_track.hpp
--- a/elasticfusion_amd/csrc/ef_track.hpp
+++ b/elasticfusion_amd/csrc/ef_track.hpp
@@ -162,7 +162,7 @@
   float icpWeight;
   Intr knext;
   bool level_changes;
-  bool split_tail;
+  int form;
 };
 int gn_update_op(const GnUpdateProbe& p, GNState* next_host, double* lastA36, double* lastb6, float* stats4);
 int track_end_tail_op(TrackState* st_host, const float* pose12, bool rgb, float weightMultiplier, double* logged16);
diff --git a/elasticfusion_amd/csrc/ef_track_host_ops.inc b/elasticfusion_amd/csrc/ef_track_host_ops.inc
--- a/elasticfusion_amd/csrc/ef_track_host_ops.inc
+++ b/elasticfusion_amd/csrc/ef_track_host_ops.inc
@@ -158,6 +158,43 @@
     __syncthreads();
   }
 }
+__global__ void __launch_bounds__(128) k_gn_update_probe_in_place(TrackState* st, const float* __restrict__ sums, const StepArgs A, int count, int sigma) {
+  __shared__ GNState gs[2];
+  __shared__ efs::SolveScratch S;
+  __shared__ float sums_s[2 * SE3_ACCS];
+  __shared__ float bg[12];
+  __shared__ int tot_s[2];
+  __shared__ unsigned char gn_member[64];
+  const int t = threadIdx.x, lane = t & 63, wave = t >> 6;
+  if (t == 0) {
+    gs[0] = st->gn[0];
+    gs[1] = st->gn[1];
+    tot_s[0] = count;
+    tot_s[1] = sigma;
+  }
+  if (t >= 64 && t < 76) bg[t - 64] = t < 73 ? st->Rprev[t - 64] : st->tprev[t - 73];
+  if (t < 64) gn_member[t] = (unsigned char)efs::gn_member_of_lane(t);
+  if (t < 2 * SE3_ACCS) sums_s[t] = sums[t];
+  __syncthreads();
+  const int cur = 0;
+  const StepArgs& H = A;
+  {
+    const int rgbSize = tot_s[0], sqsum = tot_s[1];
+    if (wave == 0) {
+      solve_step_in_place(st, &gs[cur], &gs[cur ^ 1], sums_s, H, S, bg, gn_member, rgbSize, sqsum, true);
+    } else if (wave == 1) {
+      efs::gn_stage_K(H.knext, S);
+      if (!H.rgbOnly && lane == 0) solve_step_rgb_aside(st, &gs[cur], &gs[cur ^ 1], H, rgbSize, sqsum, true);
+    }
+    __syncthreads();
+    if (S.tail_pending) {
+      if (wave == 0) efs::gn_tail_pose<true>(S, &gs[cur ^ 1], true, bg);
+      else if (wave == 1) efs::gn_tail_krk<true, true>(H.knext, S, &gs[cur ^ 1], true);
+      __syncthreads();
+    }
+  }
+  if (t == 0) st->gn[1] = gs[1];
+}
 __global__ void k_track_end_tail_probe(TrackState* st, const float* __restrict__ pose12, bool rgb, float weightMultiplier, double* traj) {
   if (threadIdx.x != 0) return;
   track_end_tail(st, pose12, pose12 + 9, rgb, weightMultiplier, traj, 0);
@@ -184,7 +221,8 @@
   if (e == hipSuccess) e = hipMemcpy(st, h, sizeof(TrackState), hipMemcpyHostToDevice);
   if (e == hipSuccess) e = hipMemcpy(sums, p.sums, sizeof(p.sums), hipMemcpyHostToDevice);
   if (e == hipSuccess) {
-    if (p.split_tail) hipLaunchKernelGGL(k_gn_update_probe<true>, dim3(1), dim3(128), 0, 0, st, (const float*)sums, A);
+    if (p.form == 2) hipLaunchKernelGGL(k_gn_update_probe_in_place, dim3(1), dim3(128), 0, 0, st, (const float*)sums, A, p.count, p.sigma);
+    else if (p.form == 1) hipLaunchKernelGGL(k_gn_update_probe<true>, dim3(1), dim3(128), 0, 0, st, (const float*)sums, A);
     else hipLaunchKernelGGL(k_gn_update_probe<false>, dim3(1), dim3(64), 0, 0, st, (const float*)sums, A);
     e = hipGetLastError();
   }
diff --git a/elasticfusion_amd/csrc/ef_track_kernels.hip b/elasticfusion_amd/csrc/ef_track_kernels.hip
--- a/elasticfusion_amd/csrc/ef_track_kernels.hip
+++ b/elasticfusion_amd/csrc/ef_track_kernels.hip
@@ -1667,22 +1667,28 @@
 }
 
 constexpr int SOLVE_BLOCK = 512;
-template <bool SPLIT_TAIL>
-__device__ __forceinline__ void solve_step_wave(TrackState* st, const GNState* prev, GNState* next, bool publish, const float* sums,
-                                                const StepArgs& A, efs::SolveScratch& S, const efs::SolvePrefetch& PF, bool stats) {
+__device__ __forceinline__ float solve_step_rgb_error(int sigma, int rgbSize) { return (float)(sqrt((double)sigma) / (rgbSize == 0 ? 1 : rgbSize)); }
+__device__ __forceinline__ void solve_step_rgb_state(TrackState* st, GNState* next, bool publish, const StepArgs& A, float rgbError, int rgbSize, bool stats) {
+  if (publish) {
+    next->rgb_broken = 0;
+    next->lastRGBErrorLevel = A.level_changes ? 3.402823466e+38f : rgbError;
+  }
+  if (stats) {
+    st->lastRGBError = rgbError;
+    st->lastRGBCount = (float)rgbSize;
+  }
+}
+__device__ __forceinline__ void solve_step_rgb_aside(TrackState* st, const GNState* prev, GNState* next, const StepArgs& A, int rgbSize, int sigma, bool stats) {
+  if (prev->rgb_broken != 0) return;
+  solve_step_rgb_state(st, next, true, A, solve_step_rgb_error(sigma, rgbSize), rgbSize, stats);
+}
+template <bool SPLIT_TAIL, bool IN_PLACE>
+__device__ __forceinline__ void solve_step_totals(TrackState* st, const GNState* prev, GNState* next, bool publish, const float* sums, const StepArgs& A,
+                                                  efs::SolveScratch& S, const efs::SolveSource src, int rgbSize, int sigma, float lastLevelErr, bool broken,
+                                                  bool stats) {
   const int lane = threadIdx.x & 63;
-  int sigma = PF.slot_b, rgbSize = PF.slot_a;
-#pragma unroll
-  for (int off = 32; off > 0; off >>= 1) {
-    rgbSize += __shfl_down(rgbSize, off, 64);
-    sigma += __shfl_down(sigma, off, 64);
-  }
-  rgbSize = __shfl(rgbSize, 0, 64);
-  sigma = __shfl(sigma, 0, 64);
-  efs::solve_prefetch_publish(PF, S);
-  const float lastLevelErr = PF.lastRGBErrorLevel;
-  const bool broken = PF.broken != 0;
-  const float rgbError = (float)(sqrt((double)sigma) / (rgbSize == 0 ? 1 : rgbSize));
+  const bool aside = IN_PLACE && !A.rgbOnly;
+  const float rgbError = aside ? 0.f : solve_step_rgb_error(sigma, rgbSize);
   const bool brk = !broken && A.rgbOnly && rgbError > lastLevelErr;
   if (broken || brk) {
     if (lane == 0) {
@@ -1708,14 +1714,9 @@
     return;
   }
   if (lane == 0) {
-    S.broken = 0;
-    if (publish) {
-      next->rgb_broken = 0;
-      next->lastRGBErrorLevel = A.level_changes ? 3.402823466e+38f : rgbError;
-    }
+    if (!IN_PLACE) S.broken = 0;
+    if (!aside) solve_step_rgb_state(st, next, publish, A, rgbError, rgbSize, stats);
     if (stats) {
-      st->lastRGBError = rgbError;
-      st->lastRGBCount = (float)rgbSize;
       if (A.icp) {
         st->lastICPError = sqrtf(sums[27]) / sums[28];
         st->lastICPCount = sums[28];
@@ -1727,7 +1728,26 @@
   }
   EF_STAMP(st, 3);
   efs::SolveInputs in{A.icp, A.rgb, A.rgbOnly, A.icpWeight, A.knext, A.level_changes};
-  efs::gauss_newton_update_wave<SPLIT_TAIL>(st, next, publish, sums, in, S, stats);
+  efs::gauss_newton_update_wave<SPLIT_TAIL, IN_PLACE>(st, next, publish, sums, in, S, stats, src);
+}
+template <bool SPLIT_TAIL>
+__device__ __forceinline__ void solve_step_wave(TrackState* st, const GNState* prev, GNState* next, bool publish, const float* sums,
+                                                const StepArgs& A, efs::SolveScratch& S, const efs::SolvePrefetch& PF, bool stats) {
+  int sigma = PF.slot_b, rgbSize = PF.slot_a;
+#pragma unroll
+  for (int off = 32; off > 0; off >>= 1) {
+    rgbSize += __shfl_down(rgbSize, off, 64);
+    sigma += __shfl_down(sigma, off, 64);
+  }
+  rgbSize = __shfl(rgbSize, 0, 64);
+  sigma = __shfl(sigma, 0, 64);
+  efs::solve_prefetch_publish(PF, S);
+  solve_step_totals<SPLIT_TAIL, false>(st, prev, next, publish, sums, A, S, efs::solve_source_of(S), rgbSize, sigma, PF.lastRGBErrorLevel, PF.broken != 0, stats);
+}
+__device__ __forceinline__ void solve_step_in_place(TrackState* st, const GNState* prev, GNState* next, const float* sums, const StepArgs& A,
+                                                    efs::SolveScratch& S, const float* prevPose, const unsigned char* member, int rgbSize, int sigma, bool stats) {
+  solve_step_totals<true, true>(st, prev, next, true, sums, A, S, efs::SolveSource{prev->resultRt, prevPose, member}, rgbSize, sigma,
+                                prev->lastRGBErrorLevel, prev->rgb_broken != 0, stats);
 }
 template <int BLOCK>
 __device__ __forceinline__ void half_partials_tree(const float* __restrict__ pairs, bool icp, bool rgb, float* sums_s) {
diff --git a/elasticfusion_amd/csrc/ef_track_ref_persistent.inc b/elasticfusion_amd/csrc/ef_track_ref_persistent.inc
--- a/elasticfusion_amd/csrc/ef_track_ref_persistent.inc
+++ b/elasticfusion_amd/csrc/ef_track_ref_persistent.inc
@@ -451,6 +451,7 @@
   __shared__ So3Loop Z;
   __shared__ int ired[2 * FT_BLOCK / 64];
   __shared__ int tot_s[2];
+  __shared__ unsigned char gn_member[64];
   __shared__ unsigned seen_a[2];
   __shared__ int dead_s;
   __shared__ unsigned mode_s;
@@ -538,6 +539,7 @@
     }
     mode_s = m;
   }
+  if (wave == 3) gn_member[lane] = (unsigned char)efs::gn_member_of_lane(lane);
   if (t == 0) {
     dead_s = (int)__hip_atomic_load(&Y->abort, __ATOMIC_RELAXED, __HIP_MEMORY_SCOPE_AGENT);
     seen_a[0] = 0u;
@@ -647,21 +649,17 @@
     }
     if (it > 0) {
       StepArgs H{true, false, HAS_ICP, HAS_RGB, false, A.icpWeight, Lv.k, lvl != ft_level_of(A.levels, it - 1), it};
-      if (t < 64) {
-        efs::SolvePrefetch PF{};
-        const GNState& gp = gs[cur];
-        PF.rt = gp.resultRt[lane & 15];
-        PF.pose = bg[lane < 12 ? lane : 0];
-        PF.slot_a = (HAS_RGB && lane == 0) ? tot_s[0] : 0;
-        PF.slot_b = (HAS_RGB && lane == 0) ? tot_s[1] : 0;
-        PF.lastRGBErrorLevel = gp.lastRGBErrorLevel;
-        PF.broken = gp.rgb_broken;
-        solve_step_wave<true>(st, &gs[cur], &gs[cur ^ 1], true, sums_s, H, S, PF, false);
+      const int rgbSize = HAS_RGB ? tot_s[0] : 0, sqsum = HAS_RGB ? tot_s[1] : 0;
+      if (wave == 0) {
+        solve_step_in_place(st, &gs[cur], &gs[cur ^ 1], sums_s, H, S, bg, gn_member, rgbSize, sqsum, false);
+      } else if (wave == 1) {
+        efs::gn_stage_K(H.knext, S);
+        if (!H.rgbOnly && lane == 0) solve_step_rgb_aside(st, &gs[cur], &gs[cur ^ 1], H, rgbSize, sqsum, false);
       }
       __syncthreads();
       if (S.tail_pending) {
-        if (wave == 0) efs::gn_tail_pose(S, &gs[cur ^ 1], true);
-        else if (wave == 1) efs::gn_tail_krk(H.knext, S, &gs[cur ^ 1], true);
+        if (wave == 0) efs::gn_tail_pose<true>(S, &gs[cur ^ 1], true, bg);
+        else if (wave == 1) efs::gn_tail_krk<true, true>(H.knext, S, &gs[cur ^ 1], true);
         __syncthreads();
       }
       FT_CLK(6);
diff --git a/include/ef_hip.h b/include/ef_hip.h
--- a/include/ef_hip.h
+++ b/include/ef_hip.h
@@ -605,7 +605,8 @@
   EF_LINALG_SE3_INVERSE_F,
   EF_LINALG_M4_AFFINE_INVERSE,
   EF_LINALG_LDLT_PIVOTS,
-  EF_LINALG_LU_INVERSE6
+  EF_LINALG_LU_INVERSE6,
+  EF_LINALG_M3_INVERSE_LANES
 };
 int ef_op_linalg(int which, const double* in_host, int n_in, double* out_host, int n_out);
 
```

New measurement: 2188 (median of 6 runs). About the same (+1.0%).
